# speechbrain/speechbrain

Hardware: AMD Instinct MI355X
Metric: audio-sec/s decoded (node), Conformer-L beam=10 (higher is better)
Workload: dtype f32

## Files before the change

### speechbrain_amd/csrc/ctc_prefix.hip

```cpp
#include "common.h"
#include "internal.h"

namespace {

constexpr float kNeg = sbk::kCtcNeg;
constexpr int kNegE = -(1 << 20);
constexpr int kHead = 24;

struct BF {
  float mg, mb;
  int eg, eb;
};

__device__ __forceinline__ float bf_log(float m, int e) {
  if (!(m > 0.0f)) return kNeg;
  const double v = ((double)e + (double)log2f(m)) * 0.69314718055994530942;
  return v < (double)kNeg ? kNeg : (float)v;
}
__device__ __forceinline__ void bf_exp(float x, float* m, int* e) {
  if (!(x > -1e19f)) {
    *m = 0.0f;
    *e = kNegE;
    return;
  }
  const double y = (double)x * 1.44269504088896340736;
  const double ip = floor(y);
  *m = exp2f((float)(y - ip));
  *e = (int)ip;
}

constexpr int kSeg = 32;
__device__ __host__ __forceinline__ int nseg_of(int T) { return (T + kSeg - 1) / kSeg; }
__device__ __host__ __forceinline__ int beam_pitch(int beam) { return 16 * ((beam + 15) / 16); }

template <typename Row>
__device__ __forceinline__ void build_segment_tables(Row row, int T, int lane, float* __restrict__ sg,
                                                     float* __restrict__ sb, int* __restrict__ se, int bp) {
  const int nseg = nseg_of(T);
  for (int s0 = 0; s0 < nseg; s0 += 2) {
    const int seg = s0 + (lane >> 5);
    const int t = seg * kSeg + (lane & 31);
    BF v{0.0f, 0.0f, kNegE, kNegE};
    if (seg < nseg && t < T) v = row(t);
    int e = max(v.mg > 0.0f ? v.eg : kNegE, v.mb > 0.0f ? v.eb : kNegE);
#pragma unroll
    for (int m = 16; m >= 1; m >>= 1) e = max(e, sbk::shfl_xor(e, m));
    if (seg < nseg && t < T) {
      sg[(size_t)t * bp] = sbk::fast_ldexp(v.mg, v.eg - e);
      sb[t] = sbk::fast_ldexp(v.mb, v.eb - e);
    }
    if (seg < nseg && (lane & 31) == 0) se[(size_t)seg * bp] = e;
  }
}

__global__ void __launch_bounds__(256) ctc_emissions_kernel(float* __restrict__ x, float* __restrict__ xb_log,
                                                            const int32_t* __restrict__ enc_len, int T, int V, int blank, int ldp) {
  const int b = blockIdx.y, t = blockIdx.x;
  float* row = x + ((size_t)b * T + t) * ldp;
  const bool pad = t >= enc_len[b];
  if (threadIdx.x == 0) xb_log[b * T + t] = pad ? (blank == 0 ? 0.0f : kNeg) : row[blank];
  __syncthreads();
  for (int c = threadIdx.x; c < V; c += 256) row[c] = pad ? (c == 0 ? 1.0f : 0.0f) : expf(row[c]);
}

__global__ void __launch_bounds__(256) ctc_init_kernel(const float* __restrict__ xb_log, BF* __restrict__ st,
                                                       float* __restrict__ sg, float* __restrict__ sb,
                                                       int* __restrict__ se, float* __restrict__ psi_prev, int T,
                                                       int beam) {
  SBK_DYN_LDS(float, cum);
  const int b = blockIdx.x;
  const int nseg = nseg_of(T);
  if (threadIdx.x == 0) {
    float c = 0.0f;
    for (int t = 0; t < T; ++t) {
      c += xb_log[b * T + t];
      cum[t] = c;
    }
  }
  __syncthreads();
  for (int t = threadIdx.x; t < T; t += 256) {
    BF v;
    bf_exp(cum[t], &v.mg, &v.eg);
    v.mb = v.mg;
    v.eb = v.eg;
    for (int j = 0; j < beam; ++j) st[((size_t)b * beam + j) * T + t] = v;
  }
  if (threadIdx.x < beam) psi_prev[b * beam + threadIdx.x] = 0.0f;
  __syncthreads();
  const int lane = threadIdx.x & 63, wave = threadIdx.x >> 6;
  for (int j = wave; j < beam; j += 4) {
    const size_t n = (size_t)b * beam + j;
    const BF* rowp = st + n * T;
    const int bp = beam_pitch(beam);
    build_segment_tables([&](int t) { return rowp[t]; }, T, lane, sg + (size_t)b * T * bp + j, sb + n * T,
                         se + (size_t)b * nseg * bp + j, bp);
  }
}

struct CtcStepArgs {
  const int32_t* last_tok;
  const int32_t* enc_len;
  int B, T, V, beam, prefix_len, blank, eos;
  float weight;
  int eos_floor;
  int use_eos_threshold;
  float eos_threshold, minus_inf;
  const int32_t* step_ptr;
  int min_steps;
  const int32_t* utt_min;
  int utt_beam, step;
  const int32_t* win;
  int window;
  int ldp;
};
__device__ __forceinline__ void ctc_frame_range(int prefix_len, int T, const int32_t* win, int window, int* start, int* end) {
  *start = prefix_len > 1 ? prefix_len : 1;
  *end = T;
  if (win) {
    *start = max(*start, win[0] - window);
    *end = min(T, win[1] + window);
  }
}
__device__ __forceinline__ int ctc_clip_to_length(int end, int blank, int len) { return blank == 0 ? min(end, max(len, 1)) : end; }

template <int NB, int TPT, bool NT>
__global__ void __launch_bounds__(256) ctc_score_step_kernel(CtcStepArgs a, const float* __restrict__ P,
                                                             const BF* __restrict__ st, const float* __restrict__ sg,
                                                             const int* __restrict__ se,
                                                             float* __restrict__ psi_out) {
  constexpr int BP = 16;
  constexpr int NV = (NB + 3) / 4;
  SBK_DYN_LDS(float, lds);
  if (a.step_ptr) a.prefix_len = a.step_ptr[0];
  const int b = blockIdx.y;
  const int j0 = blockIdx.z * BP, bp = beam_pitch(a.beam);
  const int T = a.T, V = a.V;
  int c[TPT], cc[TPT];
  bool c_ok[TPT];
#pragma unroll
  for (int k = 0; k < TPT; ++k) {
    c[k] = TPT == 4 ? (blockIdx.x * 256 + threadIdx.x) * 4 + k : (blockIdx.x * TPT + k) * 256 + threadIdx.x;
    c_ok[k] = c[k] < V;
    cc[k] = c_ok[k] ? c[k] : V - 1;
  }
  const int c4 = c_ok[0] ? c[0] : V - 4;
  const int nseg = nseg_of(T);
  int start, end;
  ctc_frame_range(a.prefix_len, T, a.win, a.window, &start, &end);
  end = ctc_clip_to_length(end, a.blank, a.enc_len[b]);
  const int ldp = a.ldp;
  const float* Pb = P + (size_t)b * T * ldp;
  const int last_frame = a.enc_len[b] - 1;
  float* tab = lds;
  int* segs = reinterpret_cast<int*>(lds + (size_t)T * BP);
  const int u_begin = start - 1, u_end = end - 1;
  if (a.win) {
    for (int i = threadIdx.x; i < nseg * BP; i += 256) {
      const int seg = i / BP, j = i % BP;
      int e = kNegE;
      if (j0 + j < a.beam) {
        const BF* row = st + (size_t)(b * a.beam + j0 + j) * T;
        for (int u = max(seg * kSeg, u_begin); u < min((seg + 1) * kSeg, u_end); ++u)
          if (row[u].mg > 0.0f) e = max(e, row[u].eg);
      }
      segs[i] = e;
    }
    __syncthreads();
    for (int i = threadIdx.x; i < T * BP; i += 256) {
      const int u = i / BP, j = i % BP;
      float v = 0.0f;
      if (j0 + j < a.beam && u >= u_begin && u < u_end) {
        const BF s = st[(size_t)(b * a.beam + j0 + j) * T + u];
        v = sbk::fast_ldexp(s.mg, (s.mg > 0.0f ? s.eg : kNegE) - segs[(u / kSeg) * BP + j]);
      }
      tab[i] = v;
    }
  } else {
    float4* dst = reinterpret_cast<float4*>(tab);
    for (int i = threadIdx.x; i < T * (BP / 4); i += 256)
      dst[i] = *reinterpret_cast<const float4*>(sg + ((size_t)b * T + i / (BP / 4)) * bp + j0 + 4 * (i % (BP / 4)));
    const int* es = se + (size_t)b * nseg * bp + j0;
    for (int i = threadIdx.x; i < nseg * BP; i += 256) segs[i] = es[(size_t)(i / BP) * bp + i % BP];
  }
  __syncthreads();

  float mps[TPT][NB];
  int Eps[TPT][NB];
  float part[TPT][NB];
#pragma unroll
  for (int k = 0; k < TPT; ++k) {
    const float p0 = Pb[cc[k]];
#pragma unroll
    for (int j = 0; j < NB; ++j) {
      const bool first = a.prefix_len == 0 && start == 1 && p0 > 0.0f;
      mps[k][j] = first ? p0 : 0.0f;
      Eps[k][j] = first ? 0 : kNegE;
      part[k][j] = 0.0f;
    }
  }
  constexpr int CH = 16 / TPT < 8 ? 8 : 16 / TPT;
  static_assert(kSeg % CH == 0, "ctc_score_step: chunks must tile a scale segment");
  auto fetch = [&](float (&buf)[TPT][CH], int cb) {
#pragma unroll
    for (int q = 0; q < CH; ++q) {
      const int u = cb + q;
      const bool ok = u >= u_begin && u < u_end;
      if constexpr (TPT == 4) {
        float4 v4 = make_float4(0.f, 0.f, 0.f, 0.f);
        if (ok) v4 = sbk::ld16<NT>(Pb + (size_t)(u + 1) * ldp + c4);
        buf[0][q] = v4.x; buf[1][q] = v4.y; buf[2][q] = v4.z; buf[3][q] = v4.w;
      } else {
#pragma unroll
        for (int k = 0; k < TPT; ++k) buf[k][q] = ok ? sbk::ld4<NT>(Pb + (size_t)(u + 1) * ldp + cc[k]) : 0.0f;
      }
    }
  };
  float nxt[TPT][CH];
  int cb = (u_begin / CH) * CH;
  if (cb < u_end) fetch(nxt, cb);
  for (; cb < u_end; cb += CH) {
    float cur[TPT][CH];
#pragma unroll
    for (int k = 0; k < TPT; ++k)
#pragma unroll
      for (int q = 0; q < CH; ++q) cur[k][q] = nxt[k][q];
    if (cb + CH < u_end) fetch(nxt, cb + CH);
#pragma unroll
    for (int q = 0; q < CH; ++q) {
      const float4* row = reinterpret_cast<const float4*>(tab + (size_t)min(cb + q, u_end - 1) * BP);
      float g[NV * 4];
#pragma unroll
      for (int v = 0; v < NV; ++v) {
        const float4 t4 = row[v];
        g[4 * v] = t4.x; g[4 * v + 1] = t4.y; g[4 * v + 2] = t4.z; g[4 * v + 3] = t4.w;
      }
#pragma unroll
      for (int k = 0; k < TPT; ++k)
#pragma unroll
        for (int j = 0; j < NB; ++j) part[k][j] = fmaf(g[j], cur[k][q], part[k][j]);
    }
    if (((cb + CH) % kSeg) == 0 || cb + CH >= u_end) {
      const int* es = segs + (cb / kSeg) * BP;
#pragma unroll
      for (int k = 0; k < TPT; ++k)
#pragma unroll
        for (int j = 0; j < NB; ++j) {
          const int kx = sbk::frexp_exp(part[k][j]);
          const int ep = part[k][j] > 0.0f ? es[j] + kx : kNegE;
          const float mp = sbk::fast_ldexp(part[k][j], -kx);
          const int P2 = max(Eps[k][j], ep);
          mps[k][j] = sbk::fast_ldexp(mps[k][j], Eps[k][j] - P2) + sbk::fast_ldexp(mp, ep - P2);
          Eps[k][j] = P2;
          part[k][j] = 0.0f;
        }
    }
  }
#pragma unroll
  for (int k = 0; k < TPT; ++k) {
    if (!c_ok[k]) continue;
#pragma unroll
    for (int j = 0; j < NB; ++j) {
      if (j0 + j < a.beam) {
        const int n = b * a.beam + j0 + j;
        float psi = bf_log(mps[k][j], Eps[k][j]);
        if (c[k] == a.eos) {
          const BF s = st[(size_t)n * T + last_frame];
          psi = bf_log(s.mg, s.eg);
        }
        if (c[k] == a.blank && a.eos != a.blank) psi = kNeg;
        psi_out[(size_t)n * V + c[k]] = psi;
      }
    }
  }
}

__global__ void __launch_bounds__(64) ctc_same_token_kernel(CtcStepArgs a, const float* __restrict__ P,
                                                            const BF* __restrict__ st, const float* __restrict__ sb,
                                                            const int* __restrict__ se, float* __restrict__ psi_out) {
  const int n = blockIdx.x, lane = threadIdx.x;
  if (a.step_ptr) a.prefix_len = a.step_ptr[0];
  const int b = n / a.beam, c = a.last_tok[n];
  const int T = a.T, V = a.V, nseg = nseg_of(T);
  if (c == a.eos || c == a.blank || c < 0 || c >= V) return;
  int start, end;
  ctc_frame_range(a.prefix_len, T, a.win, a.window, &start, &end);
  end = ctc_clip_to_length(end, a.blank, a.enc_len[b]);
  const float* Pb = P + (size_t)b * T * a.ldp;
  float m = 0.0f;
  int E = kNegE;
  if (lane == 0 && a.prefix_len == 0 && start == 1 && Pb[c] > 0.0f) {
    m = Pb[c];
    E = 0;
  }
  for (int u = start - 1 + lane; u < end - 1; u += 64) {
    const float bt = a.win ? st[(size_t)n * T + u].mb : sb[(size_t)n * T + u];
    const float term = bt * Pb[(size_t)(u + 1) * a.ldp + c];
    const int k = sbk::frexp_exp(term);
    const int eb = a.win ? st[(size_t)n * T + u].eb : se[((size_t)b * nseg + u / kSeg) * beam_pitch(a.beam) + n % a.beam];
    const int et = term > 0.0f ? eb + k : kNegE;
    const float mt = sbk::fast_ldexp(term, -k);
    const int E2 = max(E, et);
    m = sbk::fast_ldexp(m, E - E2) + sbk::fast_ldexp(mt, et - E2);
    E = E2;
  }
  int Emax = E;
#pragma unroll
  for (int k = 32; k >= 1; k >>= 1) Emax = max(Emax, sbk::shfl_xor(Emax, k));
  float v = sbk::fast_ldexp(m, E - Emax);
  v = sbk::wave_sum(v);
  if (lane == 0) psi_out[(size_t)n * V + c] = bf_log(v, Emax);
}

__global__ void __launch_bounds__(256) ctc_combine_kernel(CtcStepArgs a, const float* __restrict__ am,
                                                          const float* __restrict__ am_max,
                                                          const float* __restrict__ psi,
                                                          const float* __restrict__ psi_prev, float* __restrict__ comb,
                                                          const float* __restrict__ extra) {
  const int n = blockIdx.y;
  const int c = blockIdx.x * 256 + threadIdx.x;
  if (c >= a.V) return;
  float v = am[(size_t)n * a.V + c];
  if (c == a.eos) {
    const int step = a.step_ptr ? a.step_ptr[0] : a.step;
    const bool floor = a.utt_min ? step < a.utt_min[n / a.utt_beam] : (a.step_ptr ? step < a.min_steps : a.eos_floor);
    if (floor) v = a.minus_inf;
    if (a.use_eos_threshold && !(v > a.eos_threshold * am_max[n])) v = a.minus_inf;
  }
  if (extra) v = sbk::add_rn(v, extra[(size_t)n * a.V + c]);
  if (c == a.blank) v = kNeg;
  comb[(size_t)n * a.V + c] = sbk::score_ctc(v, psi[(size_t)n * a.V + c], psi_prev[n], a.weight);
}

struct AMap {
  float a, c, d, v0, v1;
  int ea, ec, ed, e0, e1;
};
struct AState {
  float nb, bl;
  int e;
};
__device__ __forceinline__ int clamp_e(int e) { return max(e, kNegE); }
__device__ __forceinline__ void norm1(float& x, int& e) {
  const int k = sbk::frexp_exp(x);
  x = sbk::fast_ldexp(x, -k);
  e = x > 0.0f ? clamp_e(e + k) : kNegE;
}
__device__ __forceinline__ void norm2(float& x, float& y, int& e) {
  const float m = fmaxf(x, y);
  const int k = sbk::frexp_exp(m);
  x = sbk::fast_ldexp(x, -k);
  y = sbk::fast_ldexp(y, -k);
  e = m > 0.0f ? e + k : kNegE;
}
__device__ __forceinline__ void bf_add(float& x, int& ex, float y, int ey) {
  const int ax = x > 0.0f ? ex : kNegE, ay = y > 0.0f ? ey : kNegE;
  const int E = max(ax, ay);
  x = sbk::fast_ldexp(x, ax - E) + sbk::fast_ldexp(y, ay - E);
  ex = E;
}
__device__ __forceinline__ AState apply_map(const AMap& m, const AState& s) {
  float x = m.a * s.nb, y = m.c * s.nb;
  int ex = clamp_e(m.ea + s.e), ey = clamp_e(m.ec + s.e);
  bf_add(x, ex, m.v0, m.e0);
  bf_add(y, ey, m.d * s.bl, clamp_e(m.ed + s.e));
  bf_add(y, ey, m.v1, m.e1);
  const int ax = x > 0.0f ? ex : kNegE, ay = y > 0.0f ? ey : kNegE;
  const int E = max(ax, ay);
  AState r{sbk::fast_ldexp(x, ax - E), sbk::fast_ldexp(y, ay - E), E};
  norm2(r.nb, r.bl, r.e);
  return r;
}
__device__ __forceinline__ AMap compose(const AMap& m2, const AMap& m1) {
  AMap r;
  r.a = m2.a * m1.a;
  r.ea = clamp_e(m2.ea + m1.ea);
  norm1(r.a, r.ea);
  r.d = m2.d * m1.d;
  r.ed = clamp_e(m2.ed + m1.ed);
  norm1(r.d, r.ed);
  r.c = m2.c * m1.a;
  r.ec = clamp_e(m2.ec + m1.ea);
  bf_add(r.c, r.ec, m2.d * m1.c, clamp_e(m2.ed + m1.ec));
  norm1(r.c, r.ec);
  r.v0 = m2.a * m1.v0;
  r.e0 = clamp_e(m2.ea + m1.e0);
  bf_add(r.v0, r.e0, m2.v0, m2.e0);
  norm1(r.v0, r.e0);
  r.v1 = m2.c * m1.v0;
  r.e1 = clamp_e(m2.ec + m1.e0);
  bf_add(r.v1, r.e1, m2.d * m1.v1, clamp_e(m2.ed + m1.e1));
  bf_add(r.v1, r.e1, m2.v1, m2.e1);
  norm1(r.v1, r.e1);
  return r;
}
__device__ __forceinline__ AMap frame_map(float pc, float pb, float mphi, int ephi) {
  AMap m;
  m.a = pc;
  m.ea = 0;
  norm1(m.a, m.ea);
  m.c = pb;
  m.ec = 0;
  norm1(m.c, m.ec);
  m.d = m.c;
  m.ed = m.ec;
  m.v0 = m.a * mphi;
  m.e0 = clamp_e(m.ea + ephi);
  norm1(m.v0, m.e0);
  m.v1 = 0.0f;
  m.e1 = kNegE;
  return m;
}
__device__ __forceinline__ AMap identity_map() { return AMap{1.0f, 0.0f, 1.0f, 0.0f, 0.0f, 0, kNegE, 0, kNegE, kNegE}; }
__device__ __forceinline__ AMap shfl_up_map(const AMap& m, int delta, int lane) {
  const int src = max(lane - delta, 0);
  AMap r;
  r.a = sbk::shfl(m.a, src);
  r.c = sbk::shfl(m.c, src);
  r.d = sbk::shfl(m.d, src);
  r.v0 = sbk::shfl(m.v0, src);
  r.v1 = sbk::shfl(m.v1, src);
  r.ea = sbk::shfl(m.ea, src);
  r.ec = sbk::shfl(m.ec, src);
  r.ed = sbk::shfl(m.ed, src);
  r.e0 = sbk::shfl(m.e0, src);
  r.e1 = sbk::shfl(m.e1, src);
  return r;
}

struct CtcAdvArgs {
  const float* P;
  const BF* st_old;
  const float* psi;
  const int32_t* parent;
  const int32_t* token;
  const int32_t* parent_last_tok;
  BF* st_new;
  float* sg_new;
  float* sb_new;
  int* se_new;
  float* psi_prev_new;
  int n_bh, T, V, beam, prefix_len, blank;
  const int32_t* step_ptr;
  const int32_t* win;
  int window;
  int ldp;
};

__global__ void __launch_bounds__(64) ctc_advance_kernel(CtcAdvArgs a) {
  SBK_DYN_LDS(float, lds);
  if (a.step_ptr) a.prefix_len = a.step_ptr[0];
  const int T = a.T;
  float* pc = lds;
  float* pb = pc + T;
  float* mph = pb + T;
  int* eph = reinterpret_cast<int*>(mph + T);
  float* onb = reinterpret_cast<float*>(eph + T);
  float* obl = onb + T;
  int* oe = reinterpret_cast<int*>(obl + T);
  const int n = blockIdx.x, lane = threadIdx.x;
  const int b = n / a.beam, p = a.parent[n], c = a.token[n];
  const bool same = a.parent_last_tok[p] == c;
  const float* Pb = a.P + (size_t)b * T * a.ldp;
  for (int tb = 0; tb < T; tb += 256) {
    float vpc[4], vpb[4];
    BF vs[4];
#pragma unroll
    for (int u = 0; u < 4; ++u) {
      const int t = min(tb + u * 64 + lane, T - 1);
      vpc[u] = Pb[(size_t)t * a.ldp + c];
      vpb[u] = Pb[(size_t)t * a.ldp + a.blank];
      vs[u] = a.st_old[(size_t)p * T + t];
    }
#pragma unroll
    for (int u = 0; u < 4; ++u) {
      const int t = tb + u * 64 + lane;
      if (t < T) {
        pc[t] = vpc[u];
        pb[t] = vpb[u];
        mph[t] = same ? vs[u].mb : vs[u].mg;
        eph[t] = same ? vs[u].eb : vs[u].eg;
      }
    }
  }
  __syncthreads();
  {
    int start, end;
    ctc_frame_range(a.prefix_len, T, a.win, a.window, &start, &end);
    const bool first = a.prefix_len == 0 && pc[0] > 0.0f;
    AState r0{first ? pc[0] : 0.0f, 0.0f, first ? 0 : kNegE};
    norm2(r0.nb, r0.bl, r0.e);
    const AState zero{0.0f, 0.0f, kNegE};
    const AState s0 = start == 1 ? r0 : zero;
    for (int t = lane; t < T; t += 64)
      if (t < start || t >= end) {
        onb[t] = t == 0 ? r0.nb : 0.0f;
        obl[t] = 0.0f;
        oe[t] = t == 0 ? r0.e : kNegE;
      }
    const int nfr = max(end - start, 0);
    const int fpl = (nfr + 63) / 64;
    const int f0 = min(start + lane * fpl, end), f1 = min(f0 + fpl, end);
    AMap mine = identity_map();
    for (int t = f0; t < f1; ++t) mine = compose(frame_map(pc[t], pb[t], mph[t - 1], eph[t - 1]), mine);
#pragma unroll
    for (int dlt = 1; dlt < 64; dlt <<= 1) {
      const AMap other = shfl_up_map(mine, dlt, lane);
      if (lane >= dlt) mine = compose(mine, other);
    }
    AMap pre = shfl_up_map(mine, 1, lane);
    if (lane == 0) pre = identity_map();
    AState st = apply_map(pre, s0);
    for (int t = f0; t < f1; ++t) {
      st = apply_map(frame_map(pc[t], pb[t], mph[t - 1], eph[t - 1]), st);
      onb[t] = st.nb;
      obl[t] = st.bl;
      oe[t] = st.e;
    }
  }
  __syncthreads();
  BF* bfrow = reinterpret_cast<BF*>(pc);
  for (int t0 = 0; t0 < T; t0 += 64) {
    const int t = t0 + lane;
    BF s{0.0f, 0.0f, kNegE, kNegE};
    if (t < T) {
      const float g = onb[t] + obl[t];
      const int kg = sbk::frexp_exp(g), kb = sbk::frexp_exp(obl[t]);
      s.mg = g > 0.0f ? sbk::fast_ldexp(g, 1 - kg) : 0.0f;
      s.eg = g > 0.0f ? oe[t] + kg - 1 : kNegE;
      s.mb = obl[t] > 0.0f ? sbk::fast_ldexp(obl[t], 1 - kb) : 0.0f;
      s.eb = obl[t] > 0.0f ? oe[t] + kb - 1 : kNegE;
      a.st_new[(size_t)n * T + t] = s;
    }
    __syncthreads();
    if (t < T) bfrow[t] = s;
  }
  __syncthreads();
  const int nseg = nseg_of(T);
  const int bp = beam_pitch(a.beam);
  build_segment_tables([&](int t) { return bfrow[t]; }, T, lane, a.sg_new + (size_t)b * T * bp + n % a.beam,
                       a.sb_new + (size_t)n * T, a.se_new + (size_t)b * nseg * bp + n % a.beam, bp);
  if (lane == 0) a.psi_prev_new[n] = a.psi[(size_t)p * a.V + c];
}

__global__ void __launch_bounds__(256) am_only_kernel(const float* __restrict__ am, float* __restrict__ comb, int V,
                                                      int eos, int eos_floor, int use_thr, float thr, float minus_inf,
                                                      const float* __restrict__ am_max,
                                                      const float* __restrict__ extra,
                                                      const int32_t* __restrict__ step_ptr, int min_steps,
                                                      const int32_t* __restrict__ utt_min, int beam, int step) {
  const int n = blockIdx.y;
  const int c = blockIdx.x * 256 + threadIdx.x;
  if (c >= V) return;
  float v = am[(size_t)n * V + c];
  if (c == eos) {
    if (step_ptr) step = step_ptr[0];
    if (utt_min ? step < utt_min[n / beam] : (step_ptr ? step < min_steps : eos_floor)) v = minus_inf;
    if (use_thr && !(v > thr * am_max[n])) v = minus_inf;
  }
  if (extra) v = sbk::add_rn(v, extra[(size_t)n * V + c]);
  comb[(size_t)n * V + c] = v;
}

__device__ __forceinline__ unsigned order_key(float x) {
  const unsigned u = __float_as_uint(x);
  return (u & 0x80000000u) ? ~u : (u | 0x80000000u);
}

__global__ void __launch_bounds__(256) row_kth_largest_kernel(const float* __restrict__ x, float* __restrict__ thr, int V,
                                                              int k) {
  __shared__ int cnt[4];
  __shared__ unsigned prefix_s;
  const float* xr = x + (size_t)blockIdx.x * V;
  unsigned prefix = 0;
  for (int bit = 31; bit >= 0; --bit) {
    const unsigned t = prefix | (1u << bit);
    int c = 0;
    for (int i = threadIdx.x; i < V; i += 256) c += order_key(xr[i]) >= t ? 1 : 0;
    c = (int)sbk::wave_sum((float)c);
    if ((threadIdx.x & 63) == 0) cnt[threadIdx.x >> 6] = c;
    __syncthreads();
    if (threadIdx.x == 0) prefix_s = ((cnt[0] + cnt[1]) + (cnt[2] + cnt[3])) >= k ? t : prefix;
    __syncthreads();
    prefix = prefix_s;
    __syncthreads();
  }
  if (threadIdx.x == 0) {
    const unsigned u = (prefix & 0x80000000u) ? (prefix & 0x7fffffffu) : ~prefix;
    thr[blockIdx.x] = __uint_as_float(u);
  }
}

__global__ void __launch_bounds__(256) ctc_partial_combine_kernel(float* __restrict__ comb, const float* __restrict__ thr,
                                                                  const float* __restrict__ psi,
                                                                  const float* __restrict__ psi_prev, int V, int blank,
                                                                  int eos, float weight, float minus_inf) {
  const int n = blockIdx.y;
  const int c = blockIdx.x * 256 + threadIdx.x;
  if (c >= V) return;
  const float base = comb[(size_t)n * V + c];
  float p = (base >= thr[n] || c == eos) ? psi[(size_t)n * V + c] : minus_inf;
  if (c == blank && eos != blank) p = minus_inf;
  comb[(size_t)n * V + c] = base + (p - psi_prev[n]) * weight;
}

__global__ void __launch_bounds__(256) row_max_kernel(const float* __restrict__ x, float* __restrict__ out, int V) {
  __shared__ float red[4];
  const float* xr = x + (size_t)blockIdx.x * V;
  float m = -INFINITY;
  for (int c = threadIdx.x; c < V; c += 256) m = fmaxf(m, xr[c]);
  m = sbk::wave_max(m);
  if ((threadIdx.x & 63) == 0) red[threadIdx.x >> 6] = m;
  __syncthreads();
  if (threadIdx.x == 0) out[blockIdx.x] = fmaxf(fmaxf(red[0], red[1]), fmaxf(red[2], red[3]));
}

}

namespace sbk {

namespace {
struct StateView {
  BF* st;
  float* sg;
  float* sb;
  int* se;
};
StateView view(float* base, int B, int beam, int T) {
  const size_t n_bh = (size_t)B * beam, bp = beam_pitch(beam);
  StateView v;
  v.st = reinterpret_cast<BF*>(base);
  v.sg = base + 4 * n_bh * T;
  v.sb = v.sg + (size_t)B * T * bp;
  v.se = reinterpret_cast<int*>(v.sb + n_bh * T);
  return v;
}
}

int ctc_psi_step(const float* P, const float* state, const int32_t* last_tok, const int32_t* enc_len, float* psi, int B,
                 int T, int V, int beam, int prefix_len, int blank, int eos, hipStream_t st, const int32_t* win, int window, int ldp);

size_t ctc_state_floats(int B, int beam, int T) {
  const size_t n_bh = (size_t)B * beam, bp = beam_pitch(beam);
  return 4 * n_bh * T + (size_t)B * T * bp + n_bh * T + (size_t)B * nseg_of(T) * bp + 16;
}

int ctc_prepare(float* x, float* xb_log, const int32_t* enc_len, float* state, float* psi_prev, int B, int T, int V,
                int beam, int blank, hipStream_t st, int ldp) {
  if (ldp < V) ldp = V;
  SBK_LAUNCH(ctc_emissions_kernel, dim3(T, B), dim3(256), 0, st, x, xb_log, enc_len, T, V, blank, ldp);
  int rc = launch_status("ctc_emissions");
  if (rc) return rc;
  StateView v = view(state, B, beam, T);
  if (hipMemsetAsync(v.sg, 0, (size_t)B * T * beam_pitch(beam) * sizeof(float), st) != hipSuccess) return fail(1, "ctc: memset");
  SBK_LAUNCH(ctc_init_kernel, dim3(B), dim3(256), (size_t)T * sizeof(float), st, (const float*)xb_log, v.st, v.sg, v.sb,
             v.se, psi_prev, T, beam);
  return launch_status("ctc_init");
}

int ctc_psi_step(const float* P, const float* state, const int32_t* last_tok, const int32_t* enc_len, float* psi, int B,
                 int T, int V, int beam, int prefix_len, int blank, int eos, hipStream_t st, const int32_t* win, int window, int ldp) {
  CtcStepArgs a{last_tok, enc_len, B, T, V, beam, prefix_len, blank, eos, 0.0f, 0, 0, 0.0f, 0.0f, g_step_ptr, 0};
  a.win = win;
  a.window = window;
  a.ldp = ldp < V ? V : ldp;
  const StateView v = view(const_cast<float*>(state), B, beam, T);
  ProfScope prof("ctc_score_step", 2.0 * B * beam * (double)T * V, 4.0 * B * (double)T * V + 4.0 * B * beam * V, st);
  constexpr int tpt = 1;
  dim3 grid(cdiv(V, 256 * tpt), B, beam_pitch(beam) / 16), block(256);
  const size_t lds = ((size_t)T * 16 + (size_t)((T + kSeg - 1) / kSeg) * 16) * sizeof(float);
  if (lds > 160 * 1024) return fail(SBK_EINVAL, "ctc_psi_step: T=%d frames need %zu B of LDS (max 160 KiB)", T, lds);
#define SBK_CTC_LAUNCH_NT(NB, TP, NT)                                                                                   \
  do {                                                                                                                  \
    if (lds > 64 * 1024 && SBK_ALLOW_DYN_LDS((ctc_score_step_kernel<NB, TP, NT>), lds) != hipSuccess)                    \
      return fail(SBK_EINVAL, "ctc_psi_step: cannot raise the LDS window to %zu B", lds);                               \
    SBK_LAUNCH((ctc_score_step_kernel<NB, TP, NT>), grid, block, lds, st, a, P, (const BF*)v.st, (const float*)v.sg,    \
               (const int*)v.se, psi);                                                                                  \
  } while (0)
#define SBK_CTC_LAUNCH_ONE(NB, TP)                                                                                      \
  do {                                                                                                                  \
    if (g_nt_mask & 4)                                                                                                  \
      SBK_CTC_LAUNCH_NT(NB, TP, true);                                                                                  \
    else                                                                                                                \
      SBK_CTC_LAUNCH_NT(NB, TP, false);                                                                                 \
  } while (0)
#define SBK_CTC_LAUNCH(NB) SBK_CTC_LAUNCH_ONE(NB, 1)
  if (beam == 1) {
    SBK_CTC_LAUNCH(1);
  } else if (beam <= 4) {
    SBK_CTC_LAUNCH(4);
  } else if (beam <= 10) {
    SBK_CTC_LAUNCH(10);
  } else {
    SBK_CTC_LAUNCH(16);
  }
#undef SBK_CTC_LAUNCH
#undef SBK_CTC_LAUNCH_ONE
#undef SBK_CTC_LAUNCH_NT
  int rc = launch_status("ctc_score_step");
  if (rc) return rc;
  SBK_LAUNCH(ctc_same_token_kernel, dim3(B * beam), dim3(64), 0, st, a, P, (const BF*)v.st, (const float*)v.sb,
             (const int*)v.se, psi);
  return launch_status("ctc_same_token");
}

int ctc_combine(const float* am, const float* am_max, const float* psi, const float* psi_prev, float* comb, int n_bh,
                int V, int blank, int eos, float weight, int eos_floor, int use_thr, float thr, float minus_inf,
                const float* extra, hipStream_t st, const int32_t* utt_min, int beam, int step) {
  CtcStepArgs a{nullptr, nullptr, 0, 0, V, 0, 0, blank, eos, weight, eos_floor, use_thr, thr, minus_inf, g_step_ptr,
                g_step_min_steps, utt_min, beam > 0 ? beam : 1, step};
  SBK_LAUNCH(ctc_combine_kernel, dim3(cdiv(V, 256), n_bh), dim3(256), 0, st, a, am, am_max, psi, psi_prev, comb, extra);
  return launch_status("ctc_combine");
}

int ctc_advance(const float* P, const float* state_old, const float* psi, const int32_t* parent, const int32_t* token,
                const int32_t* parent_last_tok, float* state_new, float* psi_prev_new, int n_bh, int T, int V, int beam,
                int prefix_len, int blank, hipStream_t st, const int32_t* win, int window, int ldp) {
  const StateView vo = view(const_cast<float*>(state_old), n_bh / beam, beam, T);
  const StateView vn = view(state_new, n_bh / beam, beam, T);
  CtcAdvArgs a{P, vo.st, psi, parent, token, parent_last_tok, vn.st, vn.sg, vn.sb, vn.se, psi_prev_new, n_bh, T, V, beam,
               prefix_len, blank, g_step_ptr, win, window, ldp < V ? V : ldp};
  const size_t lds = (size_t)7 * T * sizeof(float);
  if (lds > 64 * 1024) return fail(SBK_EINVAL, "ctc_advance: T=%d too long for the LDS window", T);
  ProfScope prof("ctc_advance", 14.0 * n_bh * T, 64.0 * n_bh * T, st);
  SBK_LAUNCH(ctc_advance_kernel, dim3(n_bh), dim3(64), lds, st, a);
  return launch_status("ctc_advance");
}

int am_only(const float* am, float* comb, int n_bh, int V, int eos, int eos_floor, int use_thr, float thr,
            float minus_inf, const float* am_max, const float* extra, hipStream_t st, const int32_t* utt_min, int beam,
            int step) {
  const int32_t* sp = g_step_ptr;
  const int min_steps = g_step_min_steps;
  SBK_LAUNCH(am_only_kernel, dim3(cdiv(V, 256), n_bh), dim3(256), 0, st, am, comb, V, eos, eos_floor, use_thr, thr,
             minus_inf, am_max, extra, sp, min_steps, utt_min, beam > 0 ? beam : 1, step);
  return launch_status("am_only");
}

int ctc_partial_combine(float* comb, float* thr, const float* psi, const float* psi_prev, int n_bh, int V, int k, int blank,
                        int eos, float weight, float minus_inf, hipStream_t st) {
  const int kk = k < 1 ? 1 : (k > V ? V : k);
  SBK_LAUNCH(row_kth_largest_kernel, dim3(n_bh), dim3(256), 0, st, (const float*)comb, thr, V, kk);
  SBK_LAUNCH(ctc_partial_combine_kernel, dim3(cdiv(V, 256), n_bh), dim3(256), 0, st, comb, (const float*)thr, psi, psi_prev,
             V, blank, eos, weight, minus_inf);
  return launch_status("ctc_partial_combine");
}

int row_max(const float* x, float* out, int rows, int V, hipStream_t st) {
  SBK_LAUNCH(row_max_kernel, dim3(rows), dim3(256), 0, st, x, out, V);
  return launch_status("row_max");
}

}


namespace {
__global__ void __launch_bounds__(256) ctc_score_delta_kernel(const float* __restrict__ psi, const float* __restrict__ psi_prev,
                                                              float* __restrict__ out, int V) {
  const int n = blockIdx.y, c = blockIdx.x * 256 + threadIdx.x;
  if (c < V) out[(size_t)n * V + c] = sbk::sub_rn(psi[(size_t)n * V + c], psi_prev[n]);
}
struct ScorerWs {
  float* phi[2];
  float* psi;
  float* psi_prev[2];
  float* xb;
};
size_t scorer_ws_floats(int B, int T, int V, int beam) {
  auto up = [](size_t n) { return (n + 63) & ~(size_t)63; };
  return 2 * up(sbk::ctc_state_floats(B, beam, T)) + up((size_t)B * beam * V) + 2 * up((size_t)B * beam) + up((size_t)B * T);
}
ScorerWs carve_scorer(void* ws, int B, int T, int V, int beam) {
  auto up = [](size_t n) { return (n + 63) & ~(size_t)63; };
  float* p = static_cast<float*>(ws);
  ScorerWs w;
  w.phi[0] = p, p += up(sbk::ctc_state_floats(B, beam, T));
  w.phi[1] = p, p += up(sbk::ctc_state_floats(B, beam, T));
  w.psi = p, p += up((size_t)B * beam * V);
  w.psi_prev[0] = p, p += up((size_t)B * beam);
  w.psi_prev[1] = p, p += up((size_t)B * beam);
  w.xb = p;
  return w;
}
}

extern "C" size_t sbk_ctc_scorer_workspace_bytes(int B, int T, int V, int beam) {
  if (B <= 0 || T <= 0 || V <= 0 || beam <= 0) return 0;
  return scorer_ws_floats(B, T, V, beam) * sizeof(float);
}

extern "C" int sbk_ctc_scorer_reset_f32(float* x, const int32_t* enc_len, void* ws, size_t ws_bytes, int B, int T, int V, int beam,
                                        int blank, sbk_stream_t stream) {
  if (B == 0) return 0;
  SBK_REQUIRE(x && enc_len && ws && B > 0 && T > 0 && V > 0 && beam > 0 && blank >= 0 && blank < V, "ctc_scorer_reset: bad arguments");
  SBK_REQUIRE(ws_bytes >= sbk_ctc_scorer_workspace_bytes(B, T, V, beam) && sbk::aligned16(ws) && sbk::aligned16(x),
              "ctc_scorer_reset: workspace too small (%zu B) or unaligned", ws_bytes);
  hipStream_t st = sbk::as_stream(stream);
  const ScorerWs w = carve_scorer(ws, B, T, V, beam);
  if (hipMemsetAsync(w.phi[1], 0, sbk::ctc_state_floats(B, beam, T) * sizeof(float), st) != hipSuccess)
    return sbk::fail(1, "ctc_scorer_reset: memset");
  return sbk::ctc_prepare(x, w.xb, enc_len, w.phi[0], w.psi_prev[0], B, T, V, beam, blank, st, V);
}

extern "C" int sbk_ctc_scorer_score_f32(const float* x, const int32_t* enc_len, void* ws, size_t ws_bytes, const int32_t* inp_tokens,
                                        int step, const int32_t* attn_window, int ctc_window_size, float* scores, int B, int T, int V,
                                        int beam, int blank, int eos, sbk_stream_t stream) {
  if (B == 0) return 0;
  SBK_REQUIRE(x && enc_len && ws && inp_tokens && scores && B > 0 && T > 0 && V > 0 && beam > 0 && step >= 0, "ctc_scorer_score: bad arguments");
  SBK_REQUIRE(ws_bytes >= sbk_ctc_scorer_workspace_bytes(B, T, V, beam), "ctc_scorer_score: workspace too small");
  SBK_REQUIRE(ctc_window_size >= 0 && (ctc_window_size == 0 || attn_window), "ctc_scorer_score: a window needs the {min, max} attention peaks");
  hipStream_t st = sbk::as_stream(stream);
  const ScorerWs w = carve_scorer(ws, B, T, V, beam);
  const int cur = step & 1;
  const int32_t* win = ctc_window_size > 0 ? attn_window : nullptr;
  int rc = sbk::ctc_psi_step(x, w.phi[cur], inp_tokens, enc_len, w.psi, B, T, V, beam, step, blank, eos, st, win, ctc_window_size, V);
  if (rc) return rc;
  SBK_LAUNCH(ctc_score_delta_kernel, dim3(sbk::cdiv(V, 256), B * beam), dim3(256), 0, st, (const float*)w.psi,
             (const float*)w.psi_prev[cur], scores, V);
  return sbk::launch_status("ctc_score_delta");
}

extern "C" int sbk_ctc_scorer_permute_f32(const float* x, void* ws, size_t ws_bytes, const int32_t* parent, const int32_t* token,
                                          const int32_t* parent_last_tok, int step, const int32_t* attn_window, int ctc_window_size,
                                          int B, int T, int V, int beam, int blank, sbk_stream_t stream) {
  if (B == 0) return 0;
  SBK_REQUIRE(x && ws && parent && token && parent_last_tok && B > 0 && T > 0 && V > 0 && beam > 0 && step >= 0, "ctc_scorer_permute: bad arguments");
  SBK_REQUIRE(ws_bytes >= sbk_ctc_scorer_workspace_bytes(B, T, V, beam), "ctc_scorer_permute: workspace too small");
  SBK_REQUIRE(ctc_window_size >= 0 && (ctc_window_size == 0 || attn_window), "ctc_scorer_permute: a window needs the {min, max} attention peaks");
  const ScorerWs w = carve_scorer(ws, B, T, V, beam);
  const int cur = step & 1;
  return sbk::ctc_advance(x, w.phi[cur], w.psi, parent, token, parent_last_tok, w.phi[cur ^ 1], w.psi_prev[cur ^ 1], B * beam, T, V,
                          beam, step, blank, sbk::as_stream(stream), ctc_window_size > 0 ? attn_window : nullptr, ctc_window_size, V);
}

extern "C" int sbk_prof_ctc_psi_repeat_f32(float* P_logsoftmax, const int32_t* enc_len, const int32_t* last_tok,
                                           float* psi, float* work, int B, int T, int V, int beam, int prefix_len,
                                           int iters, float* us_per_launch, sbk_stream_t stream) {
  SBK_REQUIRE(P_logsoftmax && enc_len && last_tok && psi && work && us_per_launch && iters > 0, "psi_repeat: bad arguments");
  hipStream_t st = sbk::as_stream(stream);
  float* state = work;
  float* xb = work + sbk::ctc_state_floats(B, beam, T);
  float* psi_prev = xb + (size_t)B * T;
  int rc = sbk::ctc_prepare(P_logsoftmax, xb, enc_len, state, psi_prev, B, T, V, beam, 0, st, V);
  hipEvent_t e0, e1;
  if (hipEventCreate(&e0) != hipSuccess || hipEventCreate(&e1) != hipSuccess) return sbk::fail(1, "event create");
  for (int i = 0; i < 2 && !rc; ++i)
    rc = sbk::ctc_psi_step(P_logsoftmax, state, last_tok, enc_len, psi, B, T, V, beam, prefix_len, 0, 2, st, nullptr, 0, V);
  (void)hipEventRecord(e0, st);
  for (int i = 0; i < iters && !rc; ++i)
    rc = sbk::ctc_psi_step(P_logsoftmax, state, last_tok, enc_len, psi, B, T, V, beam, prefix_len, 0, 2, st, nullptr, 0, V);
  (void)hipEventRecord(e1, st);
  (void)hipEventSynchronize(e1);
  float ms = 0.0f;
  (void)hipEventElapsedTime(&ms, e0, e1);
  *us_per_launch = ms * 1000.0f / iters;
  return rc;
}
```

### speechbrain_amd/csrc/search.hip

```cpp
#include <limits.h>

#include "common.h"
#include "internal.h"

namespace {
struct AsyncPoll {
  static constexpr int kRing = 4;
  int32_t* host = nullptr;
  hipEvent_t ev[kRing] = {};
  int issued = 0;
  bool ok = false;
  bool begin() {
    if (!ok) {
      if (hipHostMalloc(reinterpret_cast<void**>(&host), kRing * sizeof(int32_t), 0) != hipSuccess) return false;
      for (int i = 0; i < kRing; ++i)
        if (hipEventCreateWithFlags(&ev[i], hipEventDisableTiming) != hipSuccess) return false;
      ok = true;
    }
    for (int j = issued > kRing ? issued - kRing : 0; j < issued; ++j) (void)hipEventSynchronize(ev[j % kRing]);
    issued = 0;
    return true;
  }
  int poll(const int32_t* counter_dev, int target, hipStream_t st) {
    const int k = issued % kRing;
    if (hipMemcpyAsync(host + k, counter_dev, sizeof(int32_t), hipMemcpyDeviceToHost, st) != hipSuccess ||
        hipEventRecord(ev[k], st) != hipSuccess)
      return -1;
    ++issued;
    if (issued >= 3) {
      const int j = (issued - 3) % kRing;
      if (hipEventSynchronize(ev[j]) != hipSuccess) return -1;
      if (host[j] >= target) return 1;
    }
    for (int q = issued >= 2 ? issued - 2 : 0; q < issued; ++q)
      if (hipEventQuery(ev[q % kRing]) == hipSuccess && host[q % kRing] >= target) return 1;
    return 0;
  }
};
thread_local AsyncPoll g_poll;
}

namespace sbk {
int embed_pos(const int32_t* tok, const float* emb, const float* pe_row, float* x, int n, int d, float scale,
              hipStream_t st);
int self_attn_step(const float* qkv, float* kcache, float* vcache, const int32_t* kv_slot, float* out, int n, int d,
                   int H, int step, int nslot, int Lmax, hipStream_t st, const int32_t* key_tok = nullptr,
                   int key_stride = 0, int key_shift = 0, int key_first = 0, int pad_idx = 0, int group = 1);
int cross_attn_step(const float* q, const float* kv, const int32_t* enc_len, float* out, float* part, int B, int T,
                    int d, int H, int beam, hipStream_t st);
size_t cross_attn_partial_floats(int B, int T, int H, int Dh, int beam);
int log_softmax_rows(const float* x, float* out, int rows, int V, float temperature, float weight, hipStream_t st,
                     const float* bias = nullptr, const float* bias2 = nullptr, int ld = 0);
int ctc_prepare(float* x, float* xb_log, const int32_t* enc_len, float* state, float* psi_prev, int B, int T, int V,
                int beam, int blank, hipStream_t st, int ldp = 0);
size_t ctc_state_floats(int B, int beam, int T);
int ctc_psi_step(const float* P, const float* state, const int32_t* last_tok, const int32_t* enc_len, float* psi, int B,
                 int T, int V, int beam, int prefix_len, int blank, int eos, hipStream_t st, const int32_t* win = nullptr,
                 int window = 0, int ldp = 0);
int cross_attn_avg_probs(const float* q, const float* kv, const int32_t* enc_len, float* out, int n, int T, int d, int H,
                         int beam, hipStream_t st);
int ctc_combine(const float* am, const float* am_max, const float* psi, const float* psi_prev, float* comb, int n_bh,
                int V, int blank, int eos, float weight, int eos_floor, int use_thr, float thr, float minus_inf,
                const float* extra, hipStream_t st, const int32_t* utt_min = nullptr, int beam = 1, int step = 0);
int ctc_advance(const float* x, const float* phi_old, const float* psi, const int32_t* parent, const int32_t* token,
                const int32_t* parent_last_tok, float* phi_new, float* psi_prev_new, int n_bh, int T, int V, int beam,
                int prefix_len, int blank, hipStream_t st, const int32_t* win = nullptr, int window = 0, int ldp = 0);
int am_only(const float* am, float* comb, int n_bh, int V, int eos, int eos_floor, int use_thr, float thr,
            float minus_inf, const float* am_max, const float* extra, hipStream_t st, const int32_t* utt_min = nullptr,
            int beam = 1, int step = 0);
int row_max(const float* x, float* out, int rows, int V, hipStream_t st);
int ctc_partial_combine(float* comb, float* thr, const float* psi, const float* psi_prev, int n_bh, int V, int k, int blank,
                        int eos, float weight, float minus_inf, hipStream_t st);
int g_score_fused = 1;
}

namespace {

struct SideStream {
  hipStream_t s = nullptr;
  hipEvent_t fork = nullptr, join = nullptr;
};
SideStream* side_stream() {
  static thread_local SideStream ss;
  if (!ss.s) {
    if (hipStreamCreateWithFlags(&ss.s, hipStreamNonBlocking) != hipSuccess) return nullptr;
    if (hipEventCreateWithFlags(&ss.fork, hipEventDisableTiming) != hipSuccess ||
        hipEventCreateWithFlags(&ss.join, hipEventDisableTiming) != hipSuccess)
      return nullptr;
  }
  return &ss;
}

constexpr int kMaxBeam = 16;
constexpr int kMaxBeamLarge = 128;

struct Cand {
  float v;
  int i;
};
__device__ __forceinline__ bool better(float v, int i, float v2, int i2) { return v > v2 || (v == v2 && i < i2); }

template <typename Load>
__device__ __forceinline__ void block_topk(int total, int k, float* out_val, int32_t* out_idx, Load load) {
  __shared__ float lv[kMaxBeam][256];
  __shared__ int li[kMaxBeam][256];
  __shared__ float wv[4][kMaxBeam];
  __shared__ int wi[4][kMaxBeam];
  const int tid = threadIdx.x, lane = tid & 63, wave = tid >> 6;
  float vals[kMaxBeam];
  int ids[kMaxBeam];
#pragma unroll
  for (int s = 0; s < kMaxBeam; ++s) {
    vals[s] = -INFINITY;
    ids[s] = INT_MAX;
  }
  for (int e = tid; e < total; e += 256) {
    float vn;
    int id;
    load(e, vn, id);
    if (vn != vn) continue;
    if (better(vn, id, vals[kMaxBeam - 1], ids[kMaxBeam - 1])) {
      float cv = vn;
      int ci = id;
#pragma unroll
      for (int s = 0; s < kMaxBeam; ++s) {
        if (better(cv, ci, vals[s], ids[s])) {
          const float tv = vals[s];
          const int ti = ids[s];
          vals[s] = cv;
          ids[s] = ci;
          cv = tv;
          ci = ti;
        }
      }
    }
  }
#pragma unroll
  for (int s = 0; s < kMaxBeam; ++s) {
    lv[s][tid] = vals[s];
    li[s][tid] = ids[s];
  }
  int hp = 0;
  for (int r = 0; r < k; ++r) {
    float v = hp < kMaxBeam ? lv[hp][tid] : -INFINITY;
    int i = hp < kMaxBeam ? li[hp][tid] : INT_MAX;
    const int mine = i;
    sbk::wave_argmax(v, i);
    if (lane == 0) {
      wv[wave][r] = v;
      wi[wave][r] = i;
    }
    if (hp < kMaxBeam && mine == i && i != INT_MAX) ++hp;
  }
  __syncthreads();
  if (wave == 0) {
    float v = -INFINITY;
    int i = INT_MAX;
    if (lane < 4 * k) {
      v = wv[lane / k][lane % k];
      i = wi[lane / k][lane % k];
    }
    for (int r = 0; r < k; ++r) {
      float bv = v;
      int bi = i;
      sbk::wave_argmax(bv, bi);
      if (lane == 0) {
        out_val[r] = bv;
        out_idx[r] = bi;
      }
      if (i == bi && bi != INT_MAX) {
        v = -INFINITY;
        i = INT_MAX;
      }
    }
  }
}

constexpr int kTopkChunks = 16;

__global__ void __launch_bounds__(256) beam_topk_stage1_kernel(const float* __restrict__ comb,
                                                               const float* __restrict__ seq, float* __restrict__ pval,
                                                               int32_t* __restrict__ pidx, int V, int beam, float norm,
                                                               const int32_t* __restrict__ step_ptr, int step,
                                                               const int32_t* __restrict__ utt_max) {
  if (step_ptr && norm > 0.0f) norm = (float)(step_ptr[0] + 1);
  if (step_ptr) step = step_ptr[0];
  const int b = blockIdx.y, ch = blockIdx.x;
  if (utt_max && step >= utt_max[b]) return;
  const int total = beam * V;
  const int len = (total + kTopkChunks - 1) / kTopkChunks;
  const int e0 = ch * len, n = max(0, min(len, total - e0));
  const float* cb = comb + (size_t)b * total;
  const float* sq = seq + b * beam;
  block_topk(n, beam, pval + ((size_t)b * kTopkChunks + ch) * kMaxBeam, pidx + ((size_t)b * kTopkChunks + ch) * kMaxBeam,
             [&](int e, float& v, int& id) {
               id = e0 + e;
               v = sbk::score_cand(sq[id / V], cb[id], norm);
             });
}

__global__ void __launch_bounds__(256) beam_topk_stage2_kernel(const float* __restrict__ pval,
                                                               const int32_t* __restrict__ pidx,
                                                               float* __restrict__ out_val,
                                                               int32_t* __restrict__ out_idx, int beam,
                                                               const int32_t* __restrict__ step_ptr, int step,
                                                               const int32_t* __restrict__ utt_max, int nchunks) {
  const int b = blockIdx.x;
  if (step_ptr) step = step_ptr[0];
  if (utt_max && step >= utt_max[b]) return;
  const float* pv = pval + (size_t)b * kTopkChunks * kMaxBeam;
  const int32_t* pi = pidx + (size_t)b * kTopkChunks * kMaxBeam;
  block_topk(nchunks * kMaxBeam, beam, out_val + b * beam, out_idx + b * beam, [&](int e, float& v, int& id) {
    const bool ok = (e % kMaxBeam) < beam;
    v = ok ? pv[e] : -INFINITY;
    id = ok ? pi[e] : INT_MAX;
  });
  __syncthreads();
  if (threadIdx.x < beam && out_idx[b * beam + threadIdx.x] == INT_MAX) out_idx[b * beam + threadIdx.x] = 0;
}

struct ScoreArgs {
  const float* logits;
  const float* bias;
  const float* bias2;
  float* am;
  const float* psi;
  const float* psi_prev;
  const float* extra;
  const float* seq;
  float* pval;
  int32_t* pidx;
  const int32_t* step_ptr;
  const int32_t* utt_min;
  const int32_t* utt_max;
  int V, beam, step, min_steps, eos_floor, use_thr, eos, blank;
  float inv_temp, w, ctc_weight, thr, minus_inf, norm;
};

template <int NPT>
__global__ void __launch_bounds__(256) score_topk_row_kernel(ScoreArgs a) {
  __shared__ float red[4];
  __shared__ float wv[4][kMaxBeam];
  __shared__ int wi[4][kMaxBeam];
  const int n = blockIdx.x, tid = threadIdx.x, lane = tid & 63, wave = tid >> 6;
  const int V = a.V, b = n / a.beam, j = n % a.beam;
  const int step = a.step_ptr ? a.step_ptr[0] : a.step;
  if (a.utt_max && step >= a.utt_max[b]) return;
  float norm = a.norm;
  if (a.step_ptr && norm > 0.0f) norm = (float)(step + 1);
  const size_t ro = (size_t)n * V;
  float x[NPT], ps[NPT], ex[NPT];
#pragma unroll
  for (int i = 0; i < NPT; ++i) x[i] = a.logits[ro + min(tid + 256 * i, V - 1)];
  if (a.psi) {
#pragma unroll
    for (int i = 0; i < NPT; ++i) ps[i] = a.psi[ro + min(tid + 256 * i, V - 1)];
  }
  if (a.extra) {
#pragma unroll
    for (int i = 0; i < NPT; ++i) ex[i] = a.extra[ro + min(tid + 256 * i, V - 1)];
  }
  float m = -INFINITY;
#pragma unroll
  for (int i = 0; i < NPT; ++i) {
    const int c = tid + 256 * i, cl = min(c, V - 1);
    const float v = sbk::ls_logit(x[i], a.bias ? a.bias[cl] : 0.0f, a.bias2 ? a.bias2[cl] : 0.0f, a.inv_temp);
    x[i] = c < V ? v : -INFINITY;
    if (c < V) m = fmaxf(m, v);
  }
  m = sbk::wave_max(m);
  if (lane == 0) red[wave] = m;
  __syncthreads();
  m = fmaxf(fmaxf(red[0], red[1]), fmaxf(red[2], red[3]));
  __syncthreads();
  float s = 0.0f;
#pragma unroll
  for (int i = 0; i < NPT; ++i)
    if (tid + 256 * i < V) s = sbk::add_rn(s, expf(sbk::sub_rn(x[i], m)));
  s = sbk::wave_sum(s);
  if (lane == 0) red[wave] = s;
  __syncthreads();
  const float lse = sbk::add_rn(m, logf((red[0] + red[1]) + (red[2] + red[3])));
  __syncthreads();
  float am_max = -INFINITY;
#pragma unroll
  for (int i = 0; i < NPT; ++i) {
    const int c = tid + 256 * i;
    if (c < V) {
      x[i] = sbk::ls_out(x[i], lse, a.w);
      a.am[ro + c] = x[i];
      am_max = fmaxf(am_max, x[i]);
    }
  }
  if (a.use_thr) {
    am_max = sbk::wave_max(am_max);
    if (lane == 0) red[wave] = am_max;
    __syncthreads();
    am_max = fmaxf(fmaxf(red[0], red[1]), fmaxf(red[2], red[3]));
  }
  const float sq = a.seq[n];
  const float pp = a.psi ? a.psi_prev[n] : 0.0f;
  unsigned dead = 0;
  float bv = -INFINITY;
  int bi = INT_MAX;
#pragma unroll
  for (int i = 0; i < NPT; ++i) {
    const int c = tid + 256 * i;
    if (c >= V) {
      dead |= 1u << i;
      continue;
    }
    float v = x[i];
    if (c == a.eos) {
      const bool floor = a.utt_min ? step < a.utt_min[b] : (a.step_ptr ? step < a.min_steps : a.eos_floor != 0);
      if (floor) v = a.minus_inf;
      if (a.use_thr && !(v > a.thr * am_max)) v = a.minus_inf;
    }
    if (a.extra) v = sbk::add_rn(v, ex[i]);
    if (a.psi) {
      if (c == a.blank) v = sbk::kCtcNeg;
      v = sbk::score_ctc(v, ps[i], pp, a.ctc_weight);
    }
    v = sbk::score_cand(sq, v, norm);
    x[i] = v;
    if (v != v) {
      dead |= 1u << i;
      continue;
    }
    const int id = j * V + c;
    if (better(v, id, bv, bi)) {
      bv = v;
      bi = id;
    }
  }
  const int k = a.beam;
  for (int r = 0; r < k; ++r) {
    float v = bv;
    int i2 = bi;
    sbk::wave_argmax(v, i2);
    if (lane == 0) {
      wv[wave][r] = v;
      wi[wave][r] = i2;
    }
    if (bi == i2 && i2 != INT_MAX) {
      dead |= 1u << ((bi - j * V - tid) >> 8);
      bv = -INFINITY;
      bi = INT_MAX;
#pragma unroll
      for (int i = 0; i < NPT; ++i) {
        const int id = j * V + tid + 256 * i;
        if (!((dead >> i) & 1u) && better(x[i], id, bv, bi)) {
          bv = x[i];
          bi = id;
        }
      }
    }
  }
  __syncthreads();
  if (wave == 0) {
    float v = -INFINITY;
    int i2 = INT_MAX;
    if (lane < 4 * k) {
      v = wv[lane / k][lane % k];
      i2 = wi[lane / k][lane % k];
    }
    float* ov_ = a.pval + ((size_t)b * kTopkChunks + j) * kMaxBeam;
    int32_t* oi_ = a.pidx + ((size_t)b * kTopkChunks + j) * kMaxBeam;
    for (int r = 0; r < k; ++r) {
      float wbv = v;
      int wbi = i2;
      sbk::wave_argmax(wbv, wbi);
      if (lane == 0) {
        ov_[r] = wbv;
        oi_[r] = wbi;
      }
      if (i2 == wbi && wbi != INT_MAX) {
        v = -INFINITY;
        i2 = INT_MAX;
      }
    }
  }
}

__device__ __forceinline__ unsigned order_key(float v) {
  const unsigned u = __float_as_uint(v);
  return (u & 0x80000000u) ? ~u : (u | 0x80000000u);
}

__global__ void __launch_bounds__(1024) beam_topk_large_kernel(const float* __restrict__ comb,
                                                               const float* __restrict__ seq,
                                                               float* __restrict__ out_val,
                                                               int32_t* __restrict__ out_idx, int V, int beam,
                                                               float norm, const int32_t* __restrict__ step_ptr,
                                                               int step, const int32_t* __restrict__ utt_max) {
  if (step_ptr && norm > 0.0f) norm = (float)(step_ptr[0] + 1);
  if (step_ptr) step = step_ptr[0];
  if (utt_max && step >= utt_max[blockIdx.x]) return;
  __shared__ int hist[256];
  __shared__ unsigned s_prefix;
  __shared__ int s_remaining, s_count, s_eq_base;
  __shared__ int scan[1024];
  __shared__ float wv[kMaxBeamLarge];
  __shared__ int wi[kMaxBeamLarge];
  const int b = blockIdx.x, tid = threadIdx.x;
  const int total = beam * V;
  const float* cb = comb + (size_t)b * total;
  const float* sq = seq + b * beam;
  auto value = [&](int e) {
    const float x = sq[e / V] + cb[e];
    const float v = norm > 0.0f ? x / norm : x;
    return v != v ? -INFINITY : v;
  };
  if (tid == 0) {
    s_prefix = 0u;
    s_remaining = beam;
  }
  for (int pass = 0; pass < 4; ++pass) {
    const int shift = 24 - 8 * pass;
    if (tid < 256) hist[tid] = 0;
    __syncthreads();
    const unsigned prefix = s_prefix;
    for (int e = tid; e < total; e += 1024) {
      const unsigned k = order_key(value(e));
      if (pass == 0 || (k >> (shift + 8)) == prefix) atomicAdd(&hist[(k >> shift) & 255u], 1);
    }
    __syncthreads();
    if (tid == 0) {
      int rem = s_remaining, d = 255;
      for (; d > 0; --d) {
        if (hist[d] >= rem) break;
        rem -= hist[d];
      }
      s_remaining = rem;
      s_prefix = (prefix << 8) | (unsigned)d;
    }
    __syncthreads();
  }
  const unsigned thr = s_prefix;
  const int need_eq = s_remaining;
  if (tid == 0) {
    s_count = 0;
    s_eq_base = 0;
  }
  for (int i = tid; i < kMaxBeamLarge; i += 1024) {
    wv[i] = -INFINITY;
    wi[i] = INT_MAX;
  }
  __syncthreads();
  __shared__ int s_ties;
  if (tid == 0) s_ties = 0;
  __syncthreads();
  for (int e = tid; e < total; e += 1024) {
    const float v = value(e);
    const unsigned k = order_key(v);
    if (k > thr) {
      const int slot = atomicAdd(&s_count, 1);
      if (slot < kMaxBeamLarge) {
        wv[slot] = v;
        wi[slot] = e;
      }
    } else if (k == thr) {
      const int t = atomicAdd(&s_ties, 1);
      if (t < 1024) scan[t] = e;
    }
  }
  __syncthreads();
  const int n_ties = s_ties;
  if (n_ties <= 1024) {
    if (tid < n_ties) {
      const int e = scan[tid];
      int rank = 0;
      for (int q = 0; q < n_ties; ++q) rank += scan[q] < e;
      if (rank < need_eq) {
        const int slot = atomicAdd(&s_count, 1);
        if (slot < kMaxBeamLarge) {
          wv[slot] = value(e);
          wi[slot] = e;
        }
      }
    }
    __syncthreads();
  } else {
    __syncthreads();
    for (int e0 = 0; e0 < total; e0 += 1024) {
      const int e = e0 + tid;
      const int is_eq = (e < total && order_key(value(e)) == thr) ? 1 : 0;
      scan[tid] = is_eq;
      __syncthreads();
      for (int off = 1; off < 1024; off <<= 1) {
        const int add = tid >= off ? scan[tid - off] : 0;
        __syncthreads();
        scan[tid] += add;
        __syncthreads();
      }
      const int eq_rank = s_eq_base + scan[tid] - is_eq;
      if (is_eq && eq_rank < need_eq) {
        const int slot = atomicAdd(&s_count, 1);
        if (slot < kMaxBeamLarge) {
          wv[slot] = value(e);
          wi[slot] = e;
        }
      }
      __syncthreads();
      if (tid == 0) s_eq_base += scan[1023];
      __syncthreads();
      if (s_eq_base >= need_eq) break;
    }
    __syncthreads();
  }
  for (int size = 2; size <= kMaxBeamLarge; size <<= 1) {
    for (int stride = size >> 1; stride > 0; stride >>= 1) {
      if (tid < kMaxBeamLarge) {
        const int partner = tid ^ stride;
        if (partner > tid) {
          const bool desc = (tid & size) == 0;
          const bool first_better = better(wv[tid], wi[tid], wv[partner], wi[partner]);
          if (desc != first_better) {
            const float tv = wv[tid];
            const int ti = wi[tid];
            wv[tid] = wv[partner];
            wi[tid] = wi[partner];
            wv[partner] = tv;
            wi[partner] = ti;
          }
        }
      }
      __syncthreads();
    }
  }
  if (tid < beam) {
    out_val[b * beam + tid] = wv[tid];
    out_idx[b * beam + tid] = wi[tid] == INT_MAX ? 0 : wi[tid];
  }
}

struct BeamState {
  int32_t* seq[2];
  float* lp[2];
  int32_t* kv_slot[2];
  int32_t* tokens[2];
  float* seq_scores;
  float* cand_val;
  int32_t* cand_idx;
  int32_t* parent;
  int32_t* fin_count;
  int32_t* fin_seq;
  float* fin_lp;
  int32_t* fin_len;
  float* fin_score;
  int32_t* n_full;
  int pos_off;
};

__global__ void step_inc_kernel(int32_t* step) { step[0] += 1; }

__global__ void beam_init_kernel(BeamState s, int B, int beam, int bos) {
  const int n = blockIdx.x * blockDim.x + threadIdx.x;
  if (n == 0) {
    s.n_full[0] = 0;
    s.n_full[1] = 0;
  }
  if (n < B) s.fin_count[n] = 0;
  if (n >= B * beam) return;
  s.tokens[0][n] = bos;
  s.seq_scores[n] = (n % beam == 0) ? 0.0f : -INFINITY;
}

__global__ void kv_prompt_init_kernel(BeamState s, int n, int Lmax, int pos_off) {
  const int i = blockIdx.x * blockDim.x + threadIdx.x;
  if (i >= n * pos_off) return;
  const int h = i / pos_off, p = i % pos_off;
  s.kv_slot[0][(size_t)h * Lmax + p] = h;
  s.kv_slot[1][(size_t)h * Lmax + p] = h;
}
__global__ void prompt_col_kernel(const int32_t* __restrict__ prompt, int32_t* __restrict__ col, int n, int beam, int P, int p) {
  const int h = blockIdx.x * blockDim.x + threadIdx.x;
  if (h < n) col[h] = prompt[(size_t)(h / beam) * P + p];
}
__global__ void probe_pick_kernel(const float* __restrict__ probe, float* __restrict__ out, int B, int beam) {
  const int b = blockIdx.x * blockDim.x + threadIdx.x;
  if (b < B) out[b] = probe[(size_t)b * beam];
}

__device__ __forceinline__ void beam_update_body(const BeamState& s, const float* __restrict__ am, int cur, int step, int V,
                                                 int beam, int Lmax, int eos, int length_norm,
                                                 const int32_t* __restrict__ utt_max) {
  __shared__ int h_src[kMaxBeamLarge];
  __shared__ int h_dst[kMaxBeamLarge];
  __shared__ int h_n;
  const int b = blockIdx.x, tid = threadIdx.x;
  const int nxt = cur ^ 1;
  if (utt_max && step >= utt_max[b]) {
    for (int idx = tid; idx < beam * (step + 1); idx += 256) {
      const int j = idx / (step + 1), p = idx % (step + 1);
      const size_t o = ((size_t)b * beam + j) * Lmax + p;
      s.seq[nxt][o] = p < step ? s.seq[cur][o] : 0;
      s.lp[nxt][o] = p < step ? s.lp[cur][o] : 0.0f;
      s.kv_slot[nxt][o + s.pos_off] = p < step ? s.kv_slot[cur][o + s.pos_off] : b * beam + j;
    }
    if (tid < beam) {
      s.tokens[nxt][b * beam + tid] = s.tokens[cur][b * beam + tid];
      s.parent[b * beam + tid] = b * beam + tid;
    }
    return;
  }
  for (int idx = tid; idx < beam * (step + 1); idx += 256) {
    const int j = idx / (step + 1), p = idx % (step + 1);
    const int n = b * beam + j;
    const int cand = s.cand_idx[n];
    const int pred = b * beam + cand / V, tok = cand % V;
    const size_t o = (size_t)n * Lmax + p, po = (size_t)pred * Lmax + p;
    if (p < step) {
      s.seq[nxt][o] = s.seq[cur][po];
      s.lp[nxt][o] = s.lp[cur][po];
      s.kv_slot[nxt][o + s.pos_off] = s.kv_slot[cur][po + s.pos_off];
    } else {
      s.seq[nxt][o] = tok;
      s.lp[nxt][o] = am[(size_t)pred * V + tok];
      s.kv_slot[nxt][o + s.pos_off] = pred;
      s.tokens[nxt][n] = tok;
      s.parent[n] = pred;
    }
  }
  if (tid == 0) {
    int cnt = s.fin_count[b], nh = 0;
    const int before = cnt;
    for (int j = 0; j < beam; ++j) {
      const int n = b * beam + j;
      const int tok = s.cand_idx[n] % V;
      const float score = s.cand_val[n];
      if (tok == eos && cnt < beam) {
        h_src[nh] = j;
        h_dst[nh] = cnt;
        ++nh;
        s.fin_len[b * beam + cnt] = step + 1;
        s.fin_score[b * beam + cnt] = score;
        ++cnt;
      }
      s.seq_scores[n] = tok == eos ? -INFINITY : (length_norm ? score * (float)(step + 1) : score);
    }
    s.fin_count[b] = cnt;
    h_n = nh;
    if (cnt == beam && before < beam) atomicAdd(s.n_full, 1);
  }
  __syncthreads();
  for (int k = 0; k < h_n; ++k) {
    const int n = b * beam + h_src[k];
    const int cand = s.cand_idx[n];
    const int pred = b * beam + cand / V, tok = cand % V;
    const size_t fo = ((size_t)b * beam + h_dst[k]) * Lmax;
    for (int p = tid; p <= step; p += 256) {
      s.fin_seq[fo + p] = p < step ? s.seq[cur][(size_t)pred * Lmax + p] : tok;
      s.fin_lp[fo + p] = p < step ? s.lp[cur][(size_t)pred * Lmax + p] : am[(size_t)pred * V + tok];
    }
  }
}

__global__ void __launch_bounds__(256) beam_update_kernel(BeamState s, const float* __restrict__ am, int cur, int step,
                                                          int V, int beam, int Lmax, int eos, int length_norm,
                                                          const int32_t* __restrict__ step_ptr,
                                                          const int32_t* __restrict__ utt_max) {
  if (step_ptr) step = step_ptr[0];
  beam_update_body(s, am, cur, step, V, beam, Lmax, eos, length_norm, utt_max);
}

__global__ void __launch_bounds__(256) beam_merge_update_kernel(BeamState s, const float* __restrict__ pval,
                                                                const int32_t* __restrict__ pidx,
                                                                const float* __restrict__ am, int cur, int step, int V,
                                                                int beam, int Lmax, int eos, int length_norm,
                                                                const int32_t* __restrict__ step_ptr,
                                                                const int32_t* __restrict__ utt_max, int nchunks) {
  const int b = blockIdx.x;
  if (step_ptr) step = step_ptr[0];
  if (!(utt_max && step >= utt_max[b])) {
    const float* pv = pval + (size_t)b * kTopkChunks * kMaxBeam;
    const int32_t* pi = pidx + (size_t)b * kTopkChunks * kMaxBeam;
    block_topk(nchunks * kMaxBeam, beam, s.cand_val + b * beam, s.cand_idx + b * beam, [&](int e, float& v, int& id) {
      const bool ok = (e % kMaxBeam) < beam;
      v = ok ? pv[e] : -INFINITY;
      id = ok ? pi[e] : INT_MAX;
    });
    __syncthreads();
    if (threadIdx.x < beam && s.cand_idx[b * beam + threadIdx.x] == INT_MAX) s.cand_idx[b * beam + threadIdx.x] = 0;
    __syncthreads();
  }
  beam_update_body(s, am, cur, step, V, beam, Lmax, eos, length_norm, utt_max);
}

__global__ void __launch_bounds__(256) beam_finalize_kernel(BeamState s, int cur, int steps_done, int beam, int Lmax,
                                                            int Lout, int topk, int32_t* __restrict__ out_tok,
                                                            int32_t* __restrict__ out_len, float* __restrict__ out_score,
                                                            float* __restrict__ out_lp,
                                                            const int32_t* __restrict__ utt_max,
                                                            int32_t* __restrict__ out_longest) {
  if (utt_max) steps_done = min(steps_done, utt_max[blockIdx.x]);
  __shared__ float e_score[kMaxBeamLarge];
  __shared__ int e_src[kMaxBeamLarge];
  __shared__ int sel[kMaxBeamLarge];
  __shared__ int n_entries;
  const int b = blockIdx.x, tid = threadIdx.x;
  if (tid == 0) {
    int cnt = s.fin_count[b];
    for (int f = 0; f < cnt; ++f) {
      e_score[f] = s.fin_score[b * beam + f];
      e_src[f] = f;
    }
    int longest = 0;
    for (int f = 0; f < cnt; ++f) longest = max(longest, s.fin_len[b * beam + f]);
    if (steps_done > 0) {
      if (cnt < beam) longest = max(longest, steps_done);
      for (int j = 0; j < beam && cnt < beam; ++j, ++cnt) {
        e_score[cnt] = s.cand_val[b * beam + j];
        e_src[cnt] = -(j + 1);
      }
    }
    atomicMax(&s.n_full[1], longest);
    if (out_longest) out_longest[b] = longest;
    n_entries = cnt;
    for (int r = 0; r < topk; ++r) {
      int bi = -1;
      for (int e = 0; e < cnt; ++e) {
        bool used = false;
        for (int q = 0; q < r; ++q) used |= sel[q] == e;
        if (!used && (bi < 0 || e_score[e] > e_score[bi])) bi = e;
      }
      sel[r] = bi;
    }
  }
  __syncthreads();
  for (int r = 0; r < topk; ++r) {
    const int e = sel[r];
    const size_t row = (size_t)b * topk + r;
    int ntok = 0;
    if (e >= 0) ntok = e_src[e] < 0 ? steps_done : s.fin_len[b * beam + e_src[e]];
    const int len = ntok > 0 ? ntok - 1 : 0;
    if (tid == 0) {
      out_score[row] = e >= 0 ? e_score[e] : 0.0f;
      out_len[row] = len;
    }
    for (int p = tid; p < Lout; p += 256) {
      int tok = 0;
      float lp = 0.0f;
      if (e >= 0 && p < ntok) {
        const size_t o = e_src[e] < 0 ? ((size_t)b * beam + (-e_src[e] - 1)) * Lmax + p
                                      : ((size_t)b * beam + e_src[e]) * Lmax + p;
        tok = e_src[e] < 0 ? s.seq[cur][o] : s.fin_seq[o];
        lp = e_src[e] < 0 ? s.lp[cur][o] : s.fin_lp[o];
      }
      out_tok[row * Lout + p] = (topk > 1 ? p < ntok : p < len) ? tok : 0;
      out_lp[row * Lout + p] = lp;
    }
  }
}

__global__ void __launch_bounds__(256) greedy_pick_kernel(const float* __restrict__ logits, int32_t* __restrict__ tok_out,
                                                          int32_t* __restrict__ ended, int32_t* __restrict__ hyp,
                                                          float* __restrict__ score, int32_t* __restrict__ n_ended,
                                                          int V, int k, int Lmax, int eos,
                                                          const float* __restrict__ bias1,
                                                          const float* __restrict__ bias2) {
  __shared__ float wv[4];
  __shared__ int wi[4];
  __shared__ float red[4];
  __shared__ float row_lse;
  const int i = blockIdx.x, tid = threadIdx.x;
  const float* x = logits + (size_t)i * V;
  auto at = [&](int c) { return x[c] + (bias1 ? bias1[c] : 0.0f) + (bias2 ? bias2[c] : 0.0f); };
  float v = -INFINITY;
  int a = INT_MAX;
  for (int c = tid; c < V; c += 256) {
    const float xc = at(c);
    if (better(xc, c, v, a)) {
      v = xc;
      a = c;
    }
  }
#pragma unroll
  for (int m = 32; m >= 1; m >>= 1) {
    const float ov = sbk::shfl_xor(v, m);
    const int oi = sbk::shfl_xor(a, m);
    if (better(ov, oi, v, a)) {
      v = ov;
      a = oi;
    }
  }
  if ((tid & 63) == 0) {
    wv[tid >> 6] = v;
    wi[tid >> 6] = a;
  }
  __syncthreads();
  float bv = wv[0];
  int bi = wi[0];
  for (int w = 1; w < 4; ++w)
    if (better(wv[w], wi[w], bv, bi)) {
      bv = wv[w];
      bi = wi[w];
    }
  float se = 0.0f;
  for (int c = tid; c < V; c += 256) se += expf(at(c) - bv);
  se = sbk::wave_sum(se);
  if ((tid & 63) == 0) red[tid >> 6] = se;
  __syncthreads();
  if (tid == 0) {
    row_lse = logf((red[0] + red[1]) + (red[2] + red[3]));
    const int was = ended[i];
    const int now = was | (bi == eos);
    if (now && !was) atomicAdd(n_ended, 1);
    ended[i] = now;
    hyp[(size_t)i * Lmax + k] = now ? eos : bi;
    score[(size_t)i * Lmax + k] = now ? 0.0f : -row_lse;
    tok_out[i] = now ? eos : bi;
  }
}

__global__ void greedy_init_kernel(int32_t* tok, int32_t* ended, int32_t* n_ended, int32_t* kv_slot, int n, int Lmax,
                                   int bos) {
  const int i = blockIdx.x * blockDim.x + threadIdx.x;
  if (i == 0) *n_ended = 0;
  if (i >= n) return;
  tok[i] = bos;
  ended[i] = 0;
  for (int p = 0; p < Lmax; ++p) kv_slot[(size_t)i * Lmax + p] = i;
}

__global__ void __launch_bounds__(256) softmax_prob_kernel(const float* __restrict__ logits, float* __restrict__ out, int V,
                                                           int token) {
  __shared__ float red[4];
  const int i = blockIdx.x, tid = threadIdx.x;
  const float* x = logits + (size_t)i * V;
  float m = -INFINITY;
  for (int c = tid; c < V; c += 256) m = fmaxf(m, x[c]);
  m = sbk::wave_max(m);
  if ((tid & 63) == 0) red[tid >> 6] = m;
  __syncthreads();
  m = fmaxf(fmaxf(red[0], red[1]), fmaxf(red[2], red[3]));
  __syncthreads();
  float se = 0.0f;
  for (int c = tid; c < V; c += 256) se += expf(x[c] - m);
  se = sbk::wave_sum(se);
  if ((tid & 63) == 0) red[tid >> 6] = se;
  __syncthreads();
  if (tid == 0) out[i] = expf(x[token] - m) / ((red[0] + red[1]) + (red[2] + red[3]));
}

__global__ void copy_rows_kernel(const float* __restrict__ src, float* __restrict__ dst, int n, int d, long dst_stride) {
  const int i = blockIdx.x;
  for (int c = threadIdx.x; c < d; c += blockDim.x) dst[(size_t)i * dst_stride + c] = src[(size_t)i * d + c];
}

struct Carver {
  char* p;
  size_t used;
  bool dry;
  template <typename T>
  T* take(size_t n) {
    const size_t bytes = (n * sizeof(T) + 255) & ~(size_t)255;
    T* r = dry ? nullptr : reinterpret_cast<T*>(p + used);
    used += bytes;
    return r;
  }
};

struct DecoderBufs {
  float *x, *h, *qkv, *ctx, *q, *ff, *logits;
  float* splitk;
  size_t splitk_floats;
  float* xpart;
  int32_t* pbar;
  mutable int pseq;
  mutable int pgrid;
  float* ckv[64];
  float *kcache[64], *vcache[64];
};

void carve_decoder(Carver& c, DecoderBufs& d, const sbk_decoder_weights* W, int n, int B, int T, int Lmax) {
  const int dm = W->d_model;
  d.x = c.take<float>((size_t)n * dm);
  d.h = c.take<float>((size_t)n * dm);
  d.qkv = c.take<float>((size_t)n * 3 * dm);
  d.ctx = c.take<float>((size_t)n * dm);
  d.q = c.take<float>((size_t)n * dm);
  d.ff = c.take<float>((size_t)n * W->d_ffn);
  d.logits = c.take<float>((size_t)n * W->vocab);
  d.splitk_floats = (size_t)4 * n * (size_t)dm;
  d.splitk = c.take<float>(d.splitk_floats);
  d.xpart = c.take<float>(sbk::cross_attn_partial_floats(B, T, W->nhead, dm / W->nhead, n / (B > 0 ? B : 1)) + 64);
  d.pbar = c.take<int32_t>(64 + 512 + 256);
  d.pseq = 0;
  d.pgrid = 0;
  for (int l = 0; l < W->n_layers; ++l) {
    d.ckv[l] = c.take<float>((size_t)B * T * 2 * dm);
    d.kcache[l] = c.take<float>((size_t)Lmax * n * dm);
    d.vcache[l] = c.take<float>((size_t)Lmax * n * dm);
  }
}

#define SBK_HIP(expr)                                                              \
  do {                                                                             \
    hipError_t e__ = (expr);                                                       \
    if (e__ != hipSuccess) return sbk::fail((int)e__, "%s: %s", #expr, hipGetErrorString(e__)); \
  } while (0)

static inline int ctc_pitch(int V) { return (V + 31) & ~31; }

#define SBK_TRY(expr)        \
  do {                       \
    int rc__ = (expr);       \
    if (rc__) return rc__;   \
  } while (0)

int project_memory(const sbk_decoder_weights* W, const DecoderBufs& d, const float* enc, int B, int T,
                   hipStream_t st) {
  const int dm = W->d_model;
  SBK_HIP(hipMemsetAsync(d.pbar, 0, (64 + 512 + 256) * sizeof(int32_t), st));
  d.pseq = 0;
  d.pgrid = 0;
  for (int l = 0; l < W->n_layers; ++l) {
    const sbk_decoder_layer& L = W->layers[l];
    float* dst = d.ckv[l];
    int rc = -1;
    if (L.ca_kv_w3 && sbk::x3_routed(B * T, 2 * dm, dm))
      rc = sbk::gemm_nt_x3(enc, dm, L.ca_kv_w3, L.ca_in_b + dm, nullptr, 0, dst, 2 * dm, B * T, 2 * dm, dm, SBK_ACT_NONE, 1.0f,
                           nullptr, 0, st);
    if (rc == -1)
      rc = sbk::gemm_nt(enc, dm, L.ca_in_w + (size_t)dm * dm, dm, L.ca_in_b + dm, nullptr, 0, dst, 2 * dm, B * T, 2 * dm, dm,
                        SBK_ACT_NONE, 1.0f, nullptr, 0, st);
    SBK_TRY(rc);
  }
  return 0;
}

int decoder_step(const sbk_decoder_weights* W, const DecoderBufs& d, const int32_t* tokens, const int32_t* kv_slot,
                 const int32_t* enc_len, int step, int n, int B, int T, int beam, int Lmax, bool want_logits,
                 hipStream_t st) {
  const int dm = W->d_model, H = W->nhead;
  if (!sbk::g_step_ptr && sbk::persist_eligible(W, n, B, beam, Lmax)) {
    const int rc = sbk::decoder_step_persist(W, tokens, kv_slot, enc_len, d.x, d.qkv, d.ctx, d.q, d.ff, d.h, d.logits, d.kcache,
                                             d.vcache, d.ckv, d.pbar, d.pseq, &d.pgrid, step, n, B, T, beam, Lmax, want_logits, st);
    if (rc == 0) {
      ++d.pseq;
      return 0;
    }
    if (rc != -1) return rc;
  }
  const float emb_scale = W->emb_scale > 0.0f ? W->emb_scale : sqrtf((float)dm);
  SBK_TRY(sbk::embed_pos(tokens, W->emb, W->pe + (size_t)step * dm, d.x, n, dm, emb_scale, st));
  auto x3r = [&](const float* A, int lda, const uint16_t* WP, const float* b, const float* R, float* C, int N, int K, int act) -> int {
    if (!WP || !sbk::x3r_routed(n, N, K)) return -1;
    return sbk::gemm_nt_x3r(A, lda, WP, b, R, N, C, N, n, N, K, act, 1.0f, st);
  };
  auto biases_aligned = [](const sbk_decoder_layer& L) {
    return sbk::aligned16(L.sa_in_b) && sbk::aligned16(L.sa_out_b) && sbk::aligned16(L.ca_in_b) && sbk::aligned16(L.ca_out_b) &&
           sbk::aligned16(L.ff1_b) && sbk::aligned16(L.ff2_b) && sbk::aligned16(L.sa_in_bf) && sbk::aligned16(L.ca_q_bf) &&
           sbk::aligned16(L.ff1_bf);
  };
  for (int l = 0; l < W->n_layers; ++l) {
    const sbk_decoder_layer& L = W->layers[l];
    if (L.sa_in_wp && L.sa_out_wp && L.ca_q_wp && L.ca_out_wp && L.ff1_wp && L.ff2_wp && sbk::x3r_routed(n, dm, dm) &&
        sbk::x3r_routed(n, dm, W->d_ffn) && biases_aligned(L)) {
      const bool lnf = sbk::x3r_ln_routed(dm) && L.sa_in_wfp && L.sa_in_bf && L.ca_q_wfp && L.ca_q_bf && L.ff1_wfp && L.ff1_bf;
      auto ln_proj = [&](const float* g_, const float* b_, const uint16_t* WFP, const float* bfold, const uint16_t* WP, const float* bias,
                         float* C, int N, int act) -> int {
        if (lnf) return sbk::gemm_ln_nt_x3r(d.x, dm, WFP, bfold, nullptr, 0, C, N, n, N, dm, W->ln_eps, act, 1.0f, st);
        SBK_TRY(sbk::layernorm(d.x, g_, b_, d.h, n, dm, W->ln_eps, SBK_ACT_NONE, st));
        return x3r(d.h, dm, WP, bias, nullptr, C, N, dm, act);
      };
      SBK_TRY(ln_proj(L.ln1_g, L.ln1_b, L.sa_in_wfp, L.sa_in_bf, L.sa_in_wp, L.sa_in_b, d.qkv, 3 * dm, SBK_ACT_NONE));
      SBK_TRY(sbk::self_attn_step(d.qkv, d.kcache[l], d.vcache[l], kv_slot, d.ctx, n, dm, H, step, n, Lmax, st, nullptr, 0, 0,
                                  0, 0, beam));
      SBK_TRY(x3r(d.ctx, dm, L.sa_out_wp, L.sa_out_b, d.x, d.x, dm, dm, SBK_ACT_NONE));
      SBK_TRY(ln_proj(L.ln2_g, L.ln2_b, L.ca_q_wfp, L.ca_q_bf, L.ca_q_wp, L.ca_in_b, d.q, dm, SBK_ACT_NONE));
      SBK_TRY(sbk::cross_attn_step(d.q, d.ckv[l], enc_len, d.ctx, d.xpart, B, T, dm, H, beam, st));
      SBK_TRY(x3r(d.ctx, dm, L.ca_out_wp, L.ca_out_b, d.x, d.x, dm, dm, SBK_ACT_NONE));
      SBK_TRY(ln_proj(L.ln3_g, L.ln3_b, L.ff1_wfp, L.ff1_bf, L.ff1_wp, L.ff1_b, d.ff, W->d_ffn, W->ffn_act));
      SBK_TRY(x3r(d.ff, W->d_ffn, L.ff2_wp, L.ff2_b, d.x, d.x, dm, W->d_ffn, SBK_ACT_NONE));
      continue;
    }
    int frc = L.sa_in_wf ? sbk::gemm_ln_nt(d.x, dm, L.sa_in_wf, dm, L.sa_in_bf, nullptr, 0, d.qkv, 3 * dm, n, 3 * dm, dm,
                                           W->ln_eps, SBK_ACT_NONE, 1.0f, st)
                         : -1;
    if (frc > 0 || frc < -1) return frc;
    if (frc == -1) {
      SBK_TRY(sbk::layernorm(d.x, L.ln1_g, L.ln1_b, d.h, n, dm, W->ln_eps, SBK_ACT_NONE, st));
      SBK_TRY(sbk::gemm_nt_ws(d.h, dm, L.sa_in_w, dm, L.sa_in_b, nullptr, 0, d.qkv, 3 * dm, n, 3 * dm, dm, SBK_ACT_NONE,
                              1.0f, nullptr, 0, d.splitk, d.splitk_floats, st));
    }
    SBK_TRY(sbk::self_attn_step(d.qkv, d.kcache[l], d.vcache[l], kv_slot, d.ctx, n, dm, H, step, n, Lmax, st, nullptr, 0, 0,
                                0, 0, beam));
    SBK_TRY(sbk::gemm_nt_ws(d.ctx, dm, L.sa_out_w, dm, L.sa_out_b, d.x, dm, d.x, dm, n, dm, dm, SBK_ACT_NONE, 1.0f, nullptr,
                         0, d.splitk, d.splitk_floats, st));
    frc = L.ca_q_wf ? sbk::gemm_ln_nt(d.x, dm, L.ca_q_wf, dm, L.ca_q_bf, nullptr, 0, d.q, dm, n, dm, dm, W->ln_eps,
                                      SBK_ACT_NONE, 1.0f, st)
                    : -1;
    if (frc > 0 || frc < -1) return frc;
    if (frc == -1) {
      SBK_TRY(sbk::layernorm(d.x, L.ln2_g, L.ln2_b, d.h, n, dm, W->ln_eps, SBK_ACT_NONE, st));
      SBK_TRY(sbk::gemm_nt_ws(d.h, dm, L.ca_in_w, dm, L.ca_in_b, nullptr, 0, d.q, dm, n, dm, dm, SBK_ACT_NONE, 1.0f, nullptr,
                              0, d.splitk, d.splitk_floats, st));
    }
    SBK_TRY(sbk::cross_attn_step(d.q, d.ckv[l], enc_len, d.ctx, d.xpart, B, T, dm, H, beam, st));
    SBK_TRY(sbk::gemm_nt_ws(d.ctx, dm, L.ca_out_w, dm, L.ca_out_b, d.x, dm, d.x, dm, n, dm, dm, SBK_ACT_NONE, 1.0f, nullptr,
                         0, d.splitk, d.splitk_floats, st));
    frc = L.ff1_wf ? sbk::gemm_ln_nt(d.x, dm, L.ff1_wf, dm, L.ff1_bf, nullptr, 0, d.ff, W->d_ffn, n, W->d_ffn, dm, W->ln_eps,
                                     W->ffn_act, 1.0f, st)
                   : -1;
    if (frc > 0 || frc < -1) return frc;
    if (frc == -1) {
      SBK_TRY(sbk::layernorm(d.x, L.ln3_g, L.ln3_b, d.h, n, dm, W->ln_eps, SBK_ACT_NONE, st));
      SBK_TRY(sbk::gemm_nt_ws(d.h, dm, L.ff1_w, dm, L.ff1_b, nullptr, 0, d.ff, W->d_ffn, n, W->d_ffn, dm, W->ffn_act, 1.0f,
                              nullptr, 0, d.splitk, d.splitk_floats, st));
    }
    SBK_TRY(sbk::gemm_nt_ws(d.ff, W->d_ffn, L.ff2_w, W->d_ffn, L.ff2_b, d.x, dm, d.x, dm, n, dm, W->d_ffn, SBK_ACT_NONE, 1.0f,
                         nullptr, 0, d.splitk, d.splitk_floats, st));
  }
  if (want_logits && W->seq_wf) {
    const int frc = sbk::gemm_ln_nt(d.x, dm, W->seq_wf, dm, W->seq_bf, nullptr, 0, d.logits, W->vocab, n, W->vocab, dm,
                                    W->ln_eps, SBK_ACT_NONE, 1.0f, st);
    if (frc != -1) return frc;
  }
  if (want_logits && W->seq_wfp && W->seq_bf && sbk::x3r_ln_routed(dm) && sbk::x3r_routed(n, W->vocab, dm) &&
      (W->vocab < 4096 || sbk::g_x3r_ln == 2)) {
    const int rc = sbk::gemm_ln_nt_x3r(d.x, dm, W->seq_wfp, W->seq_bf, nullptr, 0, d.logits, W->vocab, n, W->vocab, dm, W->ln_eps,
                                       SBK_ACT_NONE, 1.0f, st);
    if (rc != -1) return rc;
  }
  SBK_TRY(sbk::layernorm(d.x, W->final_ln_g, W->final_ln_b, d.h, n, dm, W->ln_eps, SBK_ACT_NONE, st));
  if (want_logits) {
    int rc = x3r(d.h, dm, W->seq_wp, W->seq_b, nullptr, d.logits, W->vocab, dm, SBK_ACT_NONE);
    if (rc == -1 && W->seq_w3 && sbk::x3_routed(n, W->vocab, dm))
      rc = sbk::gemm_nt_x3(d.h, dm, W->seq_w3, W->seq_b, nullptr, 0, d.logits, W->vocab, n, W->vocab, dm, SBK_ACT_NONE, 1.0f,
                           nullptr, 0, st);
    if (rc == -1)
      rc = sbk::gemm_nt_ws(d.h, dm, W->seq_w, dm, W->seq_b, nullptr, 0, d.logits, W->vocab, n, W->vocab, dm, SBK_ACT_NONE, 1.0f,
                           nullptr, 0, d.splitk, d.splitk_floats, st);
    SBK_TRY(rc);
  }
  return 0;
}

struct LmBufs {
  float *x, *t, *h, *qkv, *ctx, *ff, *logits;
  float* splitk;
  size_t splitk_floats;
  float *kcache[64], *vcache[64];
};

void carve_lm(Carver& c, LmBufs& d, const sbk_lm_weights* LM, int n, int Lmax) {
  const int dm = LM->d_model;
  d.x = c.take<float>((size_t)n * dm);
  d.t = c.take<float>((size_t)n * dm);
  d.h = c.take<float>((size_t)n * dm);
  d.qkv = c.take<float>((size_t)n * 3 * dm);
  d.ctx = c.take<float>((size_t)n * dm);
  d.ff = c.take<float>((size_t)n * LM->d_ffn);
  d.logits = c.take<float>((size_t)n * LM->vocab);
  d.splitk_floats = (size_t)4 * n * (size_t)dm;
  d.splitk = c.take<float>(d.splitk_floats);
  for (int l = 0; l < LM->n_layers; ++l) {
    d.kcache[l] = c.take<float>((size_t)Lmax * n * dm);
    d.vcache[l] = c.take<float>((size_t)Lmax * n * dm);
  }
}

int check_lm(const sbk_lm_weights* LM) {
  SBK_REQUIRE(LM && LM->layers && LM->emb && LM->pe && LM->final_ln_g && LM->final_ln_b && LM->out0_w && LM->out0_b &&
                  LM->out_ln_g && LM->out_ln_b && LM->out2_w && LM->out2_b,
              "lm weights: null pointer");
  SBK_REQUIRE(LM->n_layers > 0 && LM->n_layers <= 64 && LM->d_model > 0 && LM->nhead > 0 &&
                  LM->d_model % LM->nhead == 0 && LM->vocab > 0,
              "lm weights: bad shape");
  return 0;
}

int lm_step(const sbk_lm_weights* LM, const LmBufs& d, const int32_t* tokens, const int32_t* kv_slot,
            const int32_t* key_tok, int key_stride, int key_shift, int key_first, int step, int n, int Lmax,
            hipStream_t st) {
  const int dm = LM->d_model, H = LM->nhead, ff = LM->d_ffn;
  const float eps = LM->ln_eps;
  auto gemm = [&](const float* A, int lda, const float* Wt, const float* b, const float* R, float* C, int N, int K,
                  int act) {
    return sbk::gemm_nt_ws(A, lda, Wt, K, b, R, R ? N : 0, C, N, n, N, K, act, 1.0f, nullptr, 0, d.splitk,
                           d.splitk_floats, st);
  };
  SBK_TRY(sbk::embed_pos(tokens, LM->emb, LM->pe + (size_t)step * dm, d.x, n, dm, sqrtf((float)dm), st));
  for (int l = 0; l < LM->n_layers; ++l) {
    const sbk_lm_layer& L = LM->layers[l];
    if (LM->normalize_before) {
      SBK_TRY(sbk::layernorm(d.x, L.ln1_g, L.ln1_b, d.h, n, dm, eps, SBK_ACT_NONE, st));
      SBK_TRY(gemm(d.h, dm, L.in_w, L.in_b, nullptr, d.qkv, 3 * dm, dm, SBK_ACT_NONE));
      SBK_TRY(sbk::self_attn_step(d.qkv, d.kcache[l], d.vcache[l], kv_slot, d.ctx, n, dm, H, step, n, Lmax, st, key_tok,
                                  key_stride, key_shift, key_first, LM->pad_idx));
      SBK_TRY(gemm(d.ctx, dm, L.out_w, L.out_b, d.x, d.x, dm, dm, SBK_ACT_NONE));
      SBK_TRY(sbk::layernorm(d.x, L.ln2_g, L.ln2_b, d.h, n, dm, eps, SBK_ACT_NONE, st));
      SBK_TRY(gemm(d.h, dm, L.ff1_w, L.ff1_b, nullptr, d.ff, ff, dm, LM->ffn_act));
      SBK_TRY(gemm(d.ff, ff, L.ff2_w, L.ff2_b, d.x, d.x, dm, ff, SBK_ACT_NONE));
    } else {
      SBK_TRY(gemm(d.x, dm, L.in_w, L.in_b, nullptr, d.qkv, 3 * dm, dm, SBK_ACT_NONE));
      SBK_TRY(sbk::self_attn_step(d.qkv, d.kcache[l], d.vcache[l], kv_slot, d.ctx, n, dm, H, step, n, Lmax, st, key_tok,
                                  key_stride, key_shift, key_first, LM->pad_idx));
      SBK_TRY(gemm(d.ctx, dm, L.out_w, L.out_b, d.x, d.t, dm, dm, SBK_ACT_NONE));
      SBK_TRY(sbk::layernorm(d.t, L.ln1_g, L.ln1_b, d.x, n, dm, eps, SBK_ACT_NONE, st));
      SBK_TRY(gemm(d.x, dm, L.ff1_w, L.ff1_b, nullptr, d.ff, ff, dm, LM->ffn_act));
      SBK_TRY(gemm(d.ff, ff, L.ff2_w, L.ff2_b, d.x, d.t, dm, ff, SBK_ACT_NONE));
      SBK_TRY(sbk::layernorm(d.t, L.ln2_g, L.ln2_b, d.x, n, dm, eps, SBK_ACT_NONE, st));
    }
  }
  SBK_TRY(sbk::layernorm(d.x, LM->final_ln_g, LM->final_ln_b, d.h, n, dm, eps, SBK_ACT_NONE, st));
  SBK_TRY(gemm(d.h, dm, LM->out0_w, LM->out0_b, nullptr, d.t, dm, dm, SBK_ACT_NONE));
  SBK_TRY(sbk::layernorm(d.t, LM->out_ln_g, LM->out_ln_b, d.h, n, dm, eps, SBK_ACT_NONE, st));
  SBK_TRY(gemm(d.h, dm, LM->out2_w, LM->out2_b, nullptr, d.logits, LM->vocab, dm, SBK_ACT_NONE));
  return 0;
}

int check_weights(const sbk_decoder_weights* W) {
  SBK_REQUIRE(W && W->layers && W->emb && W->pe && W->final_ln_g && W->final_ln_b, "decoder weights: null pointer");
  SBK_REQUIRE(W->n_layers > 0 && W->n_layers <= 64 && W->d_model > 0 && W->nhead > 0 && W->d_model % W->nhead == 0,
              "decoder weights: bad shape");
  return 0;
}

struct BeamBufs {
  BeamState s;
  float *am, *comb, *psi, *am_max, *ctc_x, *ctc_xb, *phi[2], *psi_prev[2];
  float* topk_val;
  int32_t* topk_idx;
  float* attn_avg;
  float* peak_val[2];
  int32_t* peak_pos[2];
  int32_t* win;
};

__global__ void __launch_bounds__(256) attn_peak_kernel(const float* __restrict__ probs, const float* __restrict__ old_val,
                                                        const int32_t* __restrict__ old_pos,
                                                        const int32_t* __restrict__ parent, float* __restrict__ new_val,
                                                        int32_t* __restrict__ new_pos, int32_t* __restrict__ win, int T,
                                                        int step) {
  __shared__ int lo_s[4], hi_s[4];
  const int n = blockIdx.x, tid = threadIdx.x;
  const int p = step > 0 ? parent[n] : n;
  int lo = INT_MAX, hi = INT_MIN;
  for (int t = tid; t < T; t += 256) {
    float v = step > 0 ? old_val[(size_t)p * T + t] : -1.0f;
    int pos = step > 0 ? old_pos[(size_t)p * T + t] : 0;
    const float a = probs[(size_t)n * T + t];
    if (a > v) {
      v = a;
      pos = step;
    }
    new_val[(size_t)n * T + t] = v;
    new_pos[(size_t)n * T + t] = pos;
    lo = min(lo, pos);
    hi = max(hi, pos);
  }
  for (int m = 32; m >= 1; m >>= 1) {
    lo = min(lo, sbk::shfl_xor(lo, m));
    hi = max(hi, sbk::shfl_xor(hi, m));
  }
  if ((tid & 63) == 0) {
    lo_s[tid >> 6] = lo;
    hi_s[tid >> 6] = hi;
  }
  __syncthreads();
  if (tid == 0) {
    atomicMin(&win[2 * step], min(min(lo_s[0], lo_s[1]), min(lo_s[2], lo_s[3])));
    atomicMax(&win[2 * step + 1], max(max(hi_s[0], hi_s[1]), max(hi_s[2], hi_s[3])));
  }
}
__global__ void win_init_kernel(int32_t* win, int steps) {
  const int i = blockIdx.x * blockDim.x + threadIdx.x;
  if (i < steps) {
    win[2 * i] = INT_MAX;
    win[2 * i + 1] = INT_MIN;
  }
}

void carve_beam(Carver& c, BeamBufs& b, int B, int beam, int T, int V, int Lmax, bool ctc, int window = 0) {
  const size_t n = (size_t)B * beam;
  for (int k = 0; k < 2; ++k) {
    b.s.seq[k] = c.take<int32_t>(n * Lmax);
    b.s.lp[k] = c.take<float>(n * Lmax);
    b.s.kv_slot[k] = c.take<int32_t>(n * Lmax);
    b.s.tokens[k] = c.take<int32_t>(n);
  }
  b.s.seq_scores = c.take<float>(n);
  b.s.cand_val = c.take<float>(n);
  b.s.cand_idx = c.take<int32_t>(n);
  b.s.parent = c.take<int32_t>(n);
  b.s.fin_count = c.take<int32_t>(B);
  b.s.fin_seq = c.take<int32_t>(n * Lmax);
  b.s.fin_lp = c.take<float>(n * Lmax);
  b.s.fin_len = c.take<int32_t>(n);
  b.s.fin_score = c.take<float>(n);
  b.s.n_full = c.take<int32_t>(64);
  b.am = c.take<float>(n * V);
  b.comb = c.take<float>(n * V);
  b.am_max = c.take<float>(n);
  b.topk_val = c.take<float>((size_t)B * kTopkChunks * kMaxBeam);
  b.topk_idx = c.take<int32_t>((size_t)B * kTopkChunks * kMaxBeam);
  if (ctc) {
    b.psi = c.take<float>(n * V);
    b.ctc_x = c.take<float>((size_t)B * T * ctc_pitch(V));
    b.ctc_xb = c.take<float>((size_t)B * T);
    for (int k = 0; k < 2; ++k) {
      b.phi[k] = c.take<float>(sbk::ctc_state_floats(B, beam, T));
      b.psi_prev[k] = c.take<float>(n);
    }
    if (window > 0) {
      b.attn_avg = c.take<float>(n * T);
      for (int k = 0; k < 2; ++k) {
        b.peak_val[k] = c.take<float>(n * T);
        b.peak_pos[k] = c.take<int32_t>(n * T);
      }
      b.win = c.take<int32_t>((size_t)2 * Lmax);
    }
  }
}

}

extern "C" size_t sbk_beam_search_workspace_bytes(const sbk_decoder_weights* W, const sbk_search_config* cfg, int B,
                                                  int T) {
  if (!W || !cfg) return 0;
  Carver c{nullptr, 0, true};
  DecoderBufs d;
  BeamBufs bb;
  const int Lmax = (cfg->max_steps > 0 ? cfg->max_steps : 1) + (cfg->prompt && cfg->prompt_len > 1 ? cfg->prompt_len - 1 : 0);
  carve_decoder(c, d, W, B * cfg->beam, B, T, Lmax);
  carve_beam(c, bb, B, cfg->beam, T, W->vocab, Lmax, cfg->ctc_weight > 0.0f, cfg->ctc_window_size);
  if (cfg->lm && cfg->lm_weight != 0.0f) {
    LmBufs lb;
    carve_lm(c, lb, cfg->lm, B * cfg->beam, Lmax);
  }
  return c.used + 256;
}

extern "C" int sbk_beam_search_f32(const sbk_decoder_weights* W, const sbk_search_config* cfg, const float* enc,
                                   const int32_t* enc_len, const float* ctc_w, const float* ctc_b, void* workspace,
                                   size_t workspace_bytes, int32_t* out_tokens, int32_t* out_len, float* out_score,
                                   float* out_logp, int32_t* out_max_len, int32_t* out_longest, int32_t* host_flag,
                                   int32_t* steps_run, int B, int T, sbk_stream_t stream) {
  SBK_TRY(check_weights(W));
  if (B == 0) {
    if (steps_run) *steps_run = 0;
    return 0;
  }
  SBK_REQUIRE(cfg && enc && enc_len && workspace && out_tokens && out_len && out_score && out_logp, "beam_search: null");
  SBK_REQUIRE(W->seq_w && W->seq_b, "beam_search: seq_lin weights missing");
  SBK_REQUIRE(cfg->beam >= 1 && cfg->beam <= kMaxBeamLarge, "beam_search: beam %d outside [1,%d]", cfg->beam,
              kMaxBeamLarge);
  const int pos_off = cfg->prompt && cfg->prompt_len > 1 ? cfg->prompt_len - 1 : 0;
  SBK_REQUIRE(pos_off + cfg->max_steps <= W->max_len, "beam_search: %d prompt + %d steps exceed the positional table (%d)",
              pos_off, cfg->max_steps, W->max_len);
  SBK_REQUIRE(!cfg->prompt || (cfg->prompt_len >= 1 && !(cfg->lm && cfg->lm_weight != 0.0f) && !cfg->utt_max_steps &&
                               !cfg->utt_min_steps),
              "beam_search: a token prompt excludes the LM scorer and the grouped search");
  SBK_REQUIRE(!cfg->out_probe || (cfg->probe_pos >= 0 && cfg->probe_pos <= pos_off && cfg->probe_token >= 0 &&
                                  cfg->probe_token < W->vocab), "beam_search: probe position / token out of range");
  const bool ctc = cfg->ctc_weight > 0.0f;
  const int topk = cfg->topk > 1 ? cfg->topk : 1;
  SBK_REQUIRE(topk <= cfg->beam, "beam_search: topk %d exceeds the beam %d", topk, cfg->beam);
  SBK_REQUIRE(!ctc || (ctc_w && ctc_b), "beam_search: ctc_weight > 0 needs the ctc_lin weights");
  SBK_REQUIRE(!ctc || (cfg->bos != cfg->eos && cfg->bos != cfg->blank && cfg->eos != cfg->blank),
              "Set blank, eos and bos to different indexes for joint ATT/CTC or CTC decoding");
  SBK_REQUIRE(workspace_bytes >= sbk_beam_search_workspace_bytes(W, cfg, B, T), "beam_search: workspace too small");
  SBK_REQUIRE((reinterpret_cast<uintptr_t>(workspace) & 255) == 0, "beam_search: workspace must be 256-byte aligned");
  hipStream_t st = sbk::as_stream(stream);
  const int beam = cfg->beam, V = W->vocab, n = B * beam, dm = W->d_model;
  const int Lmax = (cfg->max_steps > 0 ? cfg->max_steps : 1) + pos_off;
  if (steps_run) *steps_run = 0;
  if (B == 0) return 0;

  Carver c{static_cast<char*>(workspace), 0, false};
  DecoderBufs d;
  BeamBufs bb;
  carve_decoder(c, d, W, n, B, T, Lmax);
  carve_beam(c, bb, B, beam, T, V, Lmax, ctc, cfg->ctc_window_size);
  const sbk_lm_weights* LM = (cfg->lm && cfg->lm_weight != 0.0f) ? cfg->lm : nullptr;
  LmBufs lb;
  if (LM) {
    SBK_TRY(check_lm(LM));
    SBK_REQUIRE(LM->vocab == V, "beam_search: the LM scores %d tokens, the decoder %d", LM->vocab, V);
    SBK_REQUIRE(cfg->max_steps <= LM->max_len, "beam_search: %d steps exceed the LM positional table", cfg->max_steps);
    SBK_REQUIRE(cfg->lm_temperature > 0.0f, "beam_search: lm_temperature must be positive");
    carve_lm(c, lb, LM, n, Lmax);
  }
  const float* extra = LM ? lb.logits : nullptr;

  const int Vp = ctc_pitch(V);
  SBK_TRY(project_memory(W, d, enc, B, T, st));
  if (ctc) {
    int rc = -1;
    if (cfg->ctc_w3 && sbk::x3_routed(B * T, V, dm))
      rc = sbk::gemm_nt_x3(enc, dm, cfg->ctc_w3, ctc_b, nullptr, 0, bb.ctc_x, Vp, B * T, V, dm, SBK_ACT_NONE, 1.0f, nullptr, 0, st);
    if (rc == -1) rc = sbk::gemm_nt(enc, dm, ctc_w, dm, ctc_b, nullptr, 0, bb.ctc_x, Vp, B * T, V, dm, SBK_ACT_NONE, 1.0f, nullptr, 0, st);
    SBK_TRY(rc);
    SBK_TRY(sbk::log_softmax_rows(bb.ctc_x, bb.ctc_x, B * T, V, 1.0f, 1.0f, st, nullptr, nullptr, Vp));
    SBK_HIP(hipMemsetAsync(bb.phi[1], 0, sbk::ctc_state_floats(B, beam, T) * sizeof(float), st));
    SBK_TRY(sbk::ctc_prepare(bb.ctc_x, bb.ctc_xb, enc_len, bb.phi[0], bb.psi_prev[0], B, T, V, beam, cfg->blank, st, Vp));
  }
  bb.s.pos_off = pos_off;
  SBK_LAUNCH(beam_init_kernel, dim3(sbk::cdiv(n > B ? n : B, 256)), dim3(256), 0, st, bb.s, B, beam, cfg->bos);
  SBK_TRY(sbk::launch_status("beam_init"));
  if (pos_off > 0) {
    SBK_LAUNCH(kv_prompt_init_kernel, dim3(sbk::cdiv(n * pos_off, 256)), dim3(256), 0, st, bb.s, n, Lmax, pos_off);
    for (int p = 0; p < pos_off; ++p) {
      const bool probe = cfg->out_probe && p == cfg->probe_pos;
      SBK_LAUNCH(prompt_col_kernel, dim3(sbk::cdiv(n, 256)), dim3(256), 0, st, cfg->prompt, bb.s.tokens[1], n, beam, pos_off + 1, p);
      SBK_TRY(decoder_step(W, d, bb.s.tokens[1], bb.s.kv_slot[0], enc_len, p, n, B, T, beam, Lmax, probe, st));
      if (probe) {
        SBK_LAUNCH(softmax_prob_kernel, dim3(n), dim3(256), 0, st, (const float*)d.logits, bb.am_max, W->vocab, cfg->probe_token);
        SBK_LAUNCH(probe_pick_kernel, dim3(sbk::cdiv(B, 256)), dim3(256), 0, st, (const float*)bb.am_max, cfg->out_probe, B, beam);
      }
    }
    SBK_LAUNCH(prompt_col_kernel, dim3(sbk::cdiv(n, 256)), dim3(256), 0, st, cfg->prompt, bb.s.tokens[0], n, beam, pos_off + 1, pos_off);
    SBK_TRY(sbk::launch_status("beam_search prompt"));
  }

  const int window = ctc ? cfg->ctc_window_size : 0;
  SBK_REQUIRE(window >= 0 && (window == 0 || (!cfg->utt_max_steps && !cfg->utt_min_steps)),
              "beam_search: ctc_window_size excludes the grouped search");
  if (window > 0) {
    SBK_LAUNCH(win_init_kernel, dim3(sbk::cdiv(Lmax, 256)), dim3(256), 0, st, bb.win, Lmax);
    SBK_TRY(sbk::launch_status("ctc window"));
  }
  const float attn_w = ctc ? 1.0f - cfg->ctc_weight : 1.0f;
  SideStream* side = (ctc && cfg->overlap_ctc && window == 0) ? side_stream() : nullptr;
  const bool psi_aside = side && (cfg->overlap_ctc & 2);
  hipStream_t cst = side ? side->s : st;
  hipStream_t pst = psi_aside ? side->s : st;
  if (ctc && psi_aside) {
    SBK_HIP(hipEventRecord(side->fork, st));
    SBK_HIP(hipStreamWaitEvent(cst, side->fork, 0));
    SBK_TRY(sbk::ctc_psi_step(bb.ctc_x, bb.phi[0], bb.s.tokens[0], enc_len, bb.psi, B, T, V, beam, 0, cfg->blank,
                              cfg->eos, pst, nullptr, 0, Vp));
    SBK_HIP(hipEventRecord(side->join, cst));
  }
  int32_t* step_dev = bb.s.n_full + 2;
  auto issue_step = [&](int step, int cur, bool counter) -> int {
    SBK_TRY(decoder_step(W, d, bb.s.tokens[cur], bb.s.kv_slot[cur], enc_len, pos_off + step, n, B, T, beam, Lmax, true, st));
    if (step == 0 && cfg->out_probe && cfg->probe_pos == pos_off) {
      SBK_LAUNCH(softmax_prob_kernel, dim3(n), dim3(256), 0, st, (const float*)d.logits, bb.am_max, W->vocab, cfg->probe_token);
      SBK_LAUNCH(probe_pick_kernel, dim3(sbk::cdiv(B, 256)), dim3(256), 0, st, (const float*)bb.am_max, cfg->out_probe, B, beam);
    }
    const bool fused = sbk::g_score_fused && beam <= kMaxBeam && V <= 256 * 32 && !(ctc && cfg->ctc_candidates > 0);
    const float ls_temp = cfg->temperature_post ? 1.0f : cfg->temperature;
    const float ls_w = cfg->temperature_post ? attn_w / cfg->temperature : attn_w;
    const float* first_bias = step == 0 ? cfg->first_bias : nullptr;
    if (!fused) {
      SBK_TRY(sbk::log_softmax_rows(d.logits, bb.am, n, V, ls_temp, ls_w, st, cfg->logit_bias, first_bias));
      if (cfg->using_eos_threshold) SBK_TRY(sbk::row_max(bb.am, bb.am_max, n, V, st));
    }
    const int eos_floor = step < cfg->min_steps;
    if (LM) {
      SBK_TRY(lm_step(LM, lb, bb.s.tokens[cur], bb.s.kv_slot[cur], bb.s.seq[cur], Lmax, 1, cfg->bos, step, n, Lmax, st));
      SBK_TRY(sbk::log_softmax_rows(lb.logits, lb.logits, n, V, cfg->lm_temperature, cfg->lm_weight, st));
    }
    const int32_t* win = nullptr;
    if (window > 0) {
      SBK_TRY(sbk::cross_attn_avg_probs(d.q, d.ckv[W->n_layers - 1], enc_len, bb.attn_avg, n, T, dm, W->nhead, beam, st));
      SBK_LAUNCH(attn_peak_kernel, dim3(n), dim3(256), 0, st, (const float*)bb.attn_avg, (const float*)bb.peak_val[cur],
                 (const int32_t*)bb.peak_pos[cur], (const int32_t*)bb.s.parent, bb.peak_val[cur ^ 1], bb.peak_pos[cur ^ 1],
                 bb.win, T, step);
      SBK_TRY(sbk::launch_status("attn_peak"));
      win = bb.win + 2 * step;
    }
    if (ctc) {
      if (side && (psi_aside || step > 0)) SBK_HIP(hipStreamWaitEvent(st, side->join, 0));
      if (!psi_aside)
        SBK_TRY(sbk::ctc_psi_step(bb.ctc_x, bb.phi[cur], bb.s.tokens[cur], enc_len, bb.psi, B, T, V, beam, step,
                                  cfg->blank, cfg->eos, st, win, window, Vp));
      if (fused) {
      } else if (cfg->ctc_candidates > 0) {
        SBK_TRY(sbk::am_only(bb.am, bb.comb, n, V, cfg->eos, eos_floor, cfg->using_eos_threshold, cfg->eos_threshold,
                             cfg->minus_inf, bb.am_max, extra, st, cfg->utt_min_steps, beam, step));
        SBK_TRY(sbk::ctc_partial_combine(bb.comb, bb.topk_val, bb.psi, bb.psi_prev[cur], n, V, cfg->ctc_candidates,
                                         cfg->blank, cfg->eos, cfg->ctc_weight, cfg->minus_inf, st));
      } else {
        SBK_TRY(sbk::ctc_combine(bb.am, bb.am_max, bb.psi, bb.psi_prev[cur], bb.comb, n, V, cfg->blank, cfg->eos,
                                 cfg->ctc_weight, eos_floor, cfg->using_eos_threshold, cfg->eos_threshold,
                                 cfg->minus_inf, extra, st, cfg->utt_min_steps, beam, step));
      }
    } else if (!fused) {
      SBK_TRY(sbk::am_only(bb.am, bb.comb, n, V, cfg->eos, eos_floor, cfg->using_eos_threshold, cfg->eos_threshold,
                           cfg->minus_inf, bb.am_max, extra, st, cfg->utt_min_steps, beam, step));
    }
    const float norm = cfg->length_normalization ? (float)(step + 1) : 0.0f;
    const int32_t* sp = sbk::g_step_ptr;
    const int32_t* umax = cfg->utt_max_steps;
    if (fused) {
      sbk::ProfScope prof("score_topk", 8.0 * n * V, (ctc ? 12.0 : 8.0) * n * V, st);
      ScoreArgs a{d.logits, cfg->logit_bias, first_bias, bb.am, ctc ? bb.psi : nullptr, ctc ? bb.psi_prev[cur] : nullptr,
                  extra, bb.s.seq_scores, bb.topk_val, bb.topk_idx, sp, cfg->utt_min_steps, umax, V, beam, step,
                  cfg->min_steps, eos_floor, cfg->using_eos_threshold, cfg->eos, cfg->blank, 1.0f / ls_temp, ls_w,
                  cfg->ctc_weight, cfg->eos_threshold, cfg->minus_inf, norm};
      if (V <= 256 * 4)
        SBK_LAUNCH(score_topk_row_kernel<4>, dim3(n), dim3(256), 0, st, a);
      else if (V <= 256 * 20)
        SBK_LAUNCH(score_topk_row_kernel<20>, dim3(n), dim3(256), 0, st, a);
      else
        SBK_LAUNCH(score_topk_row_kernel<32>, dim3(n), dim3(256), 0, st, a);
    } else if (beam > kMaxBeam) {
      sbk::ProfScope prof("beam_topk_large", 10.0 * n * V, 20.0 * n * V, st);
      SBK_LAUNCH(beam_topk_large_kernel, dim3(B), dim3(1024), 0, st, (const float*)bb.comb,
                 (const float*)bb.s.seq_scores, bb.s.cand_val, bb.s.cand_idx, V, beam, norm, sp, step, umax);
    } else {
      sbk::ProfScope prof("beam_topk", 2.0 * n * V, 4.0 * n * V, st);
      SBK_LAUNCH(beam_topk_stage1_kernel, dim3(kTopkChunks, B), dim3(256), 0, st, (const float*)bb.comb,
                 (const float*)bb.s.seq_scores, bb.topk_val, bb.topk_idx, V, beam, norm, sp, step, umax);
      SBK_LAUNCH(beam_topk_stage2_kernel, dim3(B), dim3(256), 0, st, (const float*)bb.topk_val,
                 (const int32_t*)bb.topk_idx, bb.s.cand_val, bb.s.cand_idx, beam, sp, step, umax, kTopkChunks);
    }
    SBK_TRY(sbk::launch_status("beam_topk"));
    {
      sbk::ProfScope prof("beam_update", 0.0, 24.0 * n * (step + 1), st);
      if (fused)
        SBK_LAUNCH(beam_merge_update_kernel, dim3(B), dim3(256), 0, st, bb.s, (const float*)bb.topk_val,
                   (const int32_t*)bb.topk_idx, (const float*)bb.am, cur, step, V, beam, Lmax, cfg->eos,
                   cfg->length_normalization, sp, umax, beam);
      else
        SBK_LAUNCH(beam_update_kernel, dim3(B), dim3(256), 0, st, bb.s, (const float*)bb.am, cur, step, V, beam, Lmax,
                   cfg->eos, cfg->length_normalization, sp, umax);
    }
    SBK_TRY(sbk::launch_status("beam_update"));
    if (ctc && (counter || step + 1 < cfg->max_steps)) {
      if (side) {
        SBK_HIP(hipEventRecord(side->fork, st));
        SBK_HIP(hipStreamWaitEvent(cst, side->fork, 0));
      }
      SBK_TRY(sbk::ctc_advance(bb.ctc_x, bb.phi[cur], bb.psi, bb.s.parent, bb.s.tokens[cur ^ 1], bb.s.tokens[cur],
                               bb.phi[cur ^ 1], bb.psi_prev[cur ^ 1], n, T, V, beam, step, cfg->blank, cst, win, window, Vp));
      if (psi_aside)
        SBK_TRY(sbk::ctc_psi_step(bb.ctc_x, bb.phi[cur ^ 1], bb.s.tokens[cur ^ 1], enc_len, bb.psi, B, T, V, beam,
                                  step + 1, cfg->blank, cfg->eos, pst, nullptr, 0, Vp));
      if (side) SBK_HIP(hipEventRecord(side->join, cst));
    }
    if (counter) {
      SBK_LAUNCH(step_inc_kernel, dim3(1), dim3(1), 0, st, step_dev);
      SBK_TRY(sbk::launch_status("step_inc"));
    }
    return 0;
  };
  const bool polling = host_flag && cfg->check_every > 0 && g_poll.begin();
  auto poll_full = [&](int steps_done) -> int {
    if (!(polling && (steps_done % cfg->check_every == 0) && steps_done < cfg->max_steps)) return 0;
    return g_poll.poll(bb.s.n_full, B, st);
  };

  int cur = 0, steps = 0;
  int graph_mode = cfg->graph_mode;
  if (graph_mode && (side || sbk::prof_enabled() || T > 900 || cfg->max_steps < 2 || pos_off > 0 || cfg->first_bias || window > 0)) graph_mode = 0;
  if (graph_mode && sbk::persist_eligible(W, n, B, beam, Lmax)) graph_mode = 0;
  if (graph_mode) {
    struct Scope {
      ~Scope() {
        sbk::g_step_ptr = nullptr;
        if (exec) (void)hipGraphExecDestroy(exec);
        if (graph) (void)hipGraphDestroy(graph);
      }
      hipGraph_t graph = nullptr;
      hipGraphExec_t exec = nullptr;
    } scope;
    SBK_HIP(hipMemsetAsync(step_dev, 0, sizeof(int32_t), st));
    sbk::g_step_ptr = step_dev;
    sbk::g_step_min_steps = cfg->min_steps;
    if (graph_mode == 1) {
      if (hipStreamBeginCapture(st, hipStreamCaptureModeThreadLocal) == hipSuccess) {
        int rc = issue_step(0, 0, true);
        if (!rc) rc = issue_step(0, 1, true);
        const hipError_t e = hipStreamEndCapture(st, &scope.graph);
        if (rc) return rc;
        if (e != hipSuccess || hipGraphInstantiate(&scope.exec, scope.graph, nullptr, nullptr, 0) != hipSuccess) {
          scope.exec = nullptr;
          (void)hipGetLastError();
        }
      } else {
        (void)hipGetLastError();
      }
    }
    const int pairs = cfg->max_steps / 2;
    bool done = false;
    for (int p = 0; p < pairs && !done; ++p) {
      if (scope.exec) {
        SBK_HIP(hipGraphLaunch(scope.exec, st));
      } else {
        SBK_TRY(issue_step(0, 0, true));
        SBK_TRY(issue_step(0, 1, true));
      }
      steps += 2;
      const int r = poll_full(steps);
      if (r < 0) return sbk::fail(1, "beam_search: stop-rule poll failed");
      done = r == 1;
    }
    if (!done && (cfg->max_steps & 1)) {
      SBK_TRY(issue_step(0, 0, true));
      ++steps;
    }
    cur = steps & 1;
  } else {
    for (int step = 0; step < cfg->max_steps; ++step) {
      SBK_TRY(issue_step(step, cur, false));
      cur ^= 1;
      steps = step + 1;
      const int r = poll_full(steps);
      if (r < 0) return sbk::fail(1, "beam_search: stop-rule poll failed");
      if (r == 1) break;
    }
  }
  if (side) SBK_HIP(hipStreamWaitEvent(st, side->join, 0));
  if (steps_run) *steps_run = steps;
  SBK_LAUNCH(beam_finalize_kernel, dim3(B), dim3(256), 0, st, bb.s, cur, steps, beam, Lmax, Lmax - pos_off, topk, out_tokens, out_len,
             out_score, out_logp, cfg->utt_max_steps, out_longest);
  SBK_TRY(sbk::launch_status("beam_finalize"));
  if (out_max_len)
    SBK_HIP(hipMemcpyAsync(out_max_len, bb.s.n_full + 1, sizeof(int32_t), hipMemcpyDeviceToDevice, st));
  return 0;
}

extern "C" size_t sbk_decoder_prefix_workspace_bytes(const sbk_decoder_weights* W, int n, int T, int L) {
  if (!W) return 0;
  Carver c{nullptr, 0, true};
  DecoderBufs d;
  carve_decoder(c, d, W, n, n, T, L);
  c.take<int32_t>((size_t)n * L);
  c.take<int32_t>((size_t)n);
  c.take<int32_t>(64 + 2 * (size_t)n);
  return c.used + 256;
}

__global__ void gather_col_kernel(const int32_t* __restrict__ tokens, int32_t* __restrict__ col, int n, int L, int p) {
  const int i = blockIdx.x * blockDim.x + threadIdx.x;
  if (i < n) col[i] = tokens[(size_t)i * L + p];
}

extern "C" int sbk_decoder_prefix_f32(const sbk_decoder_weights* W, const int32_t* tokens, const float* enc,
                                      const int32_t* enc_len, void* workspace, size_t workspace_bytes, float* pred,
                                      int n, int T, int L, sbk_stream_t stream) {
  SBK_TRY(check_weights(W));
  if (n == 0 || L == 0) return 0;
  SBK_REQUIRE(tokens && enc && enc_len && workspace && pred, "decoder_prefix: null");
  SBK_REQUIRE(L <= W->max_len, "decoder_prefix: prefix longer than the positional table");
  SBK_REQUIRE(workspace_bytes >= sbk_decoder_prefix_workspace_bytes(W, n, T, L), "decoder_prefix: workspace too small");
  hipStream_t st = sbk::as_stream(stream);
  if (n == 0 || L == 0) return 0;
  Carver c{static_cast<char*>(workspace), 0, false};
  DecoderBufs d;
  carve_decoder(c, d, W, n, n, T, L);
  int32_t* kv_slot = c.take<int32_t>((size_t)n * L);
  int32_t* col = c.take<int32_t>((size_t)n);
  int32_t* misc = c.take<int32_t>(64 + 2 * (size_t)n);
  SBK_TRY(project_memory(W, d, enc, n, T, st));
  SBK_LAUNCH(greedy_init_kernel, dim3(sbk::cdiv(n, 256)), dim3(256), 0, st, misc + 64, misc + 64 + n, misc, kv_slot, n, L, 0);
  SBK_TRY(sbk::launch_status("prefix_init"));
  for (int p = 0; p < L; ++p) {
    SBK_LAUNCH(gather_col_kernel, dim3(sbk::cdiv(n, 256)), dim3(256), 0, st, tokens, col, n, L, p);
    SBK_TRY(decoder_step(W, d, col, kv_slot, enc_len, p, n, n, T, 1, L, false, st));
    SBK_LAUNCH(copy_rows_kernel, dim3(n), dim3(256), 0, st, (const float*)d.h, pred + (size_t)p * W->d_model, n,
               W->d_model, (long)L * W->d_model);
    SBK_TRY(sbk::launch_status("prefix_copy"));
  }
  return 0;
}

extern "C" size_t sbk_lm_prefix_workspace_bytes(const sbk_lm_weights* LM, int n, int L) {
  if (!LM) return 0;
  Carver c{nullptr, 0, true};
  LmBufs d;
  carve_lm(c, d, LM, n, L > 0 ? L : 1);
  c.take<int32_t>((size_t)n * (L > 0 ? L : 1));
  c.take<int32_t>((size_t)n);
  c.take<int32_t>(64 + 2 * (size_t)n);
  return c.used + 256;
}

extern "C" int sbk_lm_prefix_f32(const sbk_lm_weights* LM, const int32_t* tokens, void* workspace,
                                 size_t workspace_bytes, float* logits, int n, int L, sbk_stream_t stream) {
  SBK_TRY(check_lm(LM));
  if (n == 0 || L == 0) return 0;
  SBK_REQUIRE(tokens && workspace && logits, "lm_prefix: null");
  SBK_REQUIRE(L <= LM->max_len, "lm_prefix: prefix longer than the positional table");
  SBK_REQUIRE(workspace_bytes >= sbk_lm_prefix_workspace_bytes(LM, n, L), "lm_prefix: workspace too small");
  hipStream_t st = sbk::as_stream(stream);
  if (n == 0 || L == 0) return 0;
  Carver c{static_cast<char*>(workspace), 0, false};
  LmBufs d;
  carve_lm(c, d, LM, n, L);
  int32_t* kv_slot = c.take<int32_t>((size_t)n * L);
  int32_t* col = c.take<int32_t>((size_t)n);
  int32_t* misc = c.take<int32_t>(64 + 2 * (size_t)n);
  SBK_LAUNCH(greedy_init_kernel, dim3(sbk::cdiv(n, 256)), dim3(256), 0, st, misc + 64, misc + 64 + n, misc, kv_slot, n, L, 0);
  SBK_TRY(sbk::launch_status("lm_prefix_init"));
  for (int p = 0; p < L; ++p) {
    SBK_LAUNCH(gather_col_kernel, dim3(sbk::cdiv(n, 256)), dim3(256), 0, st, tokens, col, n, L, p);
    SBK_TRY(lm_step(LM, d, col, kv_slot, tokens, L, 0, 0, p, n, L, st));
    SBK_LAUNCH(copy_rows_kernel, dim3(n), dim3(256), 0, st, (const float*)d.logits, logits + (size_t)p * LM->vocab, n,
               LM->vocab, (long)L * LM->vocab);
    SBK_TRY(sbk::launch_status("lm_prefix_copy"));
  }
  return 0;
}

extern "C" size_t sbk_greedy_search_workspace_bytes(const sbk_decoder_weights* W, int B, int T, int max_steps) {
  if (!W) return 0;
  Carver c{nullptr, 0, true};
  DecoderBufs d;
  const int L = max_steps > 0 ? max_steps : 1;
  carve_decoder(c, d, W, B, B, T, L);
  c.take<int32_t>((size_t)B * L);
  c.take<int32_t>(64 + 2 * (size_t)B);
  return c.used + 256;
}

extern "C" int sbk_greedy_search_f32(const sbk_decoder_weights* W, const float* enc, const int32_t* enc_len,
                                     void* workspace, size_t workspace_bytes, int32_t* out_tokens, float* out_scores,
                                     int32_t* host_flag, int32_t* steps_run, int B, int T, int min_steps, int max_steps,
                                     int bos, int eos, int check_every, sbk_stream_t stream) {
  SBK_TRY(check_weights(W));
  if (B == 0) {
    if (steps_run) *steps_run = 0;
    return 0;
  }
  SBK_REQUIRE(enc && enc_len && workspace && out_tokens && out_scores && W->seq_w && W->seq_b, "greedy_search: null");
  SBK_REQUIRE(max_steps <= W->max_len, "greedy_search: too many steps for the positional table");
  SBK_REQUIRE(workspace_bytes >= sbk_greedy_search_workspace_bytes(W, B, T, max_steps), "greedy: workspace too small");
  hipStream_t st = sbk::as_stream(stream);
  if (steps_run) *steps_run = 0;
  const int L = max_steps > 0 ? max_steps : 1;
  if (B == 0) return 0;
  Carver c{static_cast<char*>(workspace), 0, false};
  DecoderBufs d;
  carve_decoder(c, d, W, B, B, T, L);
  int32_t* kv_slot = c.take<int32_t>((size_t)B * L);
  int32_t* misc = c.take<int32_t>(64 + 2 * (size_t)B);
  int32_t *n_ended = misc, *tok = misc + 64, *ended = misc + 64 + B;
  SBK_TRY(project_memory(W, d, enc, B, T, st));
  SBK_LAUNCH(greedy_init_kernel, dim3(sbk::cdiv(B, 256)), dim3(256), 0, st, tok, ended, n_ended, kv_slot, B, L, bos);
  SBK_TRY(sbk::launch_status("greedy_init"));
  SBK_HIP(hipMemsetAsync(out_tokens, 0, (size_t)B * L * sizeof(int32_t), st));
  SBK_HIP(hipMemsetAsync(out_scores, 0, (size_t)B * L * sizeof(float), st));
  int k = 0;
  const bool polling = host_flag && check_every > 0 && g_poll.begin();
  for (int step = min_steps; step < max_steps; ++step, ++k) {
    SBK_TRY(decoder_step(W, d, tok, kv_slot, enc_len, k, B, B, T, 1, L, true, st));
    SBK_LAUNCH(greedy_pick_kernel, dim3(B), dim3(256), 0, st, (const float*)d.logits, tok, ended, out_tokens,
               out_scores, n_ended, W->vocab, k, L, eos, (const float*)nullptr, (const float*)nullptr);
    SBK_TRY(sbk::launch_status("greedy_pick"));
    if (polling && ((k + 1) % check_every == 0)) {
      const int r = g_poll.poll(n_ended, B, st);
      if (r < 0) return sbk::fail(1, "greedy_search: stop-rule poll failed");
      if (r == 1) {
        ++k;
        break;
      }
    }
  }
  if (steps_run) *steps_run = k;
  return 0;
}

extern "C" size_t sbk_prompted_greedy_search_workspace_bytes(const sbk_decoder_weights* W, int B, int T, int P,
                                                             int max_new) {
  if (!W) return 0;
  Carver c{nullptr, 0, true};
  DecoderBufs d;
  const int L = (P > 0 ? P - 1 : 0) + (max_new > 0 ? max_new : 1);
  carve_decoder(c, d, W, B, B, T, L);
  c.take<int32_t>((size_t)B * L);
  c.take<int32_t>((size_t)B);
  c.take<int32_t>(64 + 2 * (size_t)B);
  return c.used + 256;
}

extern "C" int sbk_prompted_greedy_search_f32(const sbk_decoder_weights* W, const float* enc, const int32_t* enc_len,
                                              const int32_t* prompt, int P, const float* logit_bias,
                                              const float* first_bias, void* workspace, size_t workspace_bytes,
                                              int32_t* out_tokens, float* out_scores, int probe_pos, int probe_token,
                                              float* out_probe, int32_t* host_flag, int32_t* steps_run, int B, int T,
                                              int max_new, int eos, int check_every, sbk_stream_t stream) {
  SBK_TRY(check_weights(W));
  if (steps_run) *steps_run = 0;
  if (B == 0 || max_new <= 0) return 0;
  SBK_REQUIRE(enc && enc_len && prompt && workspace && out_tokens && out_scores && W->seq_w && W->seq_b,
              "prompted_greedy_search: null");
  SBK_REQUIRE(P >= 1, "prompted_greedy_search: the prompt holds at least the first decoder input token");
  const int L = P - 1 + max_new;
  SBK_REQUIRE(L <= W->max_len, "prompted_greedy_search: prompt + new tokens (%d) exceed the positional table (%d)", L,
              W->max_len);
  SBK_REQUIRE(!out_probe || (probe_pos >= 0 && probe_pos < P && probe_token >= 0 && probe_token < W->vocab),
              "prompted_greedy_search: probe position / token out of range");
  SBK_REQUIRE(workspace_bytes >= sbk_prompted_greedy_search_workspace_bytes(W, B, T, P, max_new),
              "prompted_greedy_search: workspace too small");
  hipStream_t st = sbk::as_stream(stream);
  Carver c{static_cast<char*>(workspace), 0, false};
  DecoderBufs d;
  carve_decoder(c, d, W, B, B, T, L);
  int32_t* kv_slot = c.take<int32_t>((size_t)B * L);
  int32_t* col = c.take<int32_t>((size_t)B);
  int32_t* misc = c.take<int32_t>(64 + 2 * (size_t)B);
  int32_t *n_ended = misc, *tok = misc + 64, *ended = misc + 64 + B;
  SBK_TRY(project_memory(W, d, enc, B, T, st));
  SBK_LAUNCH(greedy_init_kernel, dim3(sbk::cdiv(B, 256)), dim3(256), 0, st, tok, ended, n_ended, kv_slot, B, L, 0);
  SBK_TRY(sbk::launch_status("greedy_init"));
  SBK_HIP(hipMemsetAsync(out_tokens, 0, (size_t)B * max_new * sizeof(int32_t), st));
  SBK_HIP(hipMemsetAsync(out_scores, 0, (size_t)B * max_new * sizeof(float), st));
  for (int p = 0; p + 1 < P; ++p) {
    const bool probe = out_probe && p == probe_pos;
    SBK_LAUNCH(gather_col_kernel, dim3(sbk::cdiv(B, 256)), dim3(256), 0, st, prompt, col, B, P, p);
    SBK_TRY(decoder_step(W, d, col, kv_slot, enc_len, p, B, B, T, 1, L, probe, st));
    if (probe) SBK_LAUNCH(softmax_prob_kernel, dim3(B), dim3(256), 0, st, (const float*)d.logits, out_probe, W->vocab, probe_token);
  }
  SBK_LAUNCH(gather_col_kernel, dim3(sbk::cdiv(B, 256)), dim3(256), 0, st, prompt, tok, B, P, P - 1);
  SBK_TRY(sbk::launch_status("prompt"));
  int k = 0;
  const bool polling = host_flag && check_every > 0 && g_poll.begin();
  for (; k < max_new; ++k) {
    SBK_TRY(decoder_step(W, d, tok, kv_slot, enc_len, P - 1 + k, B, B, T, 1, L, true, st));
    if (k == 0 && out_probe && probe_pos == P - 1)
      SBK_LAUNCH(softmax_prob_kernel, dim3(B), dim3(256), 0, st, (const float*)d.logits, out_probe, W->vocab, probe_token);
    SBK_LAUNCH(greedy_pick_kernel, dim3(B), dim3(256), 0, st, (const float*)d.logits, tok, ended, out_tokens, out_scores,
               n_ended, W->vocab, k, max_new, eos, logit_bias, k == 0 ? first_bias : (const float*)nullptr);
    SBK_TRY(sbk::launch_status("greedy_pick"));
    if (polling && ((k + 1) % check_every == 0)) {
      const int r = g_poll.poll(n_ended, B, st);
      if (r < 0) return sbk::fail(1, "greedy_search: stop-rule poll failed");
      if (r == 1) {
        ++k;
        break;
      }
    }
  }
  if (steps_run) *steps_run = k < max_new ? k : max_new;
  return 0;
}
```

Measured before the change: 13070.

## Fuse same-token CTC score into advance and drop full am write in fused scorer

The CTC advance kernel now also builds segment tables in LDS and computes the repeated-token prefix score for the next step, so the separate same-token kernel launch per step is removed and psi_step patches that entry from a small buffer. The fused score/top-k kernel gains a TAIL mode that skips writing the full log-prob row and instead stores only the selected candidates' acoustic scores, which beam update then reads. TAIL is enabled by default by raising g_score_fused to 2. This trades one kernel launch and an n*V store per step for extra LDS work in advance and recomputing log-softmax for the winning candidates.

```diff
diff --git a/speechbrain_amd/csrc/ctc_prefix.hip b/speechbrain_amd/csrc/ctc_prefix.hip
--- a/speechbrain_amd/csrc/ctc_prefix.hip
+++ b/speechbrain_amd/csrc/ctc_prefix.hip
@@ -35,7 +35,8 @@
 
 template <typename Row>
 __device__ __forceinline__ void build_segment_tables(Row row, int T, int lane, float* __restrict__ sg,
-                                                     float* __restrict__ sb, int* __restrict__ se, int bp) {
+                                                     float* __restrict__ sb, int* __restrict__ se, int bp,
+                                                     float* lds_sb = nullptr, int* lds_se = nullptr) {
   const int nseg = nseg_of(T);
   for (int s0 = 0; s0 < nseg; s0 += 2) {
     const int seg = s0 + (lane >> 5);
@@ -47,9 +48,14 @@
     for (int m = 16; m >= 1; m >>= 1) e = max(e, sbk::shfl_xor(e, m));
     if (seg < nseg && t < T) {
       sg[(size_t)t * bp] = sbk::fast_ldexp(v.mg, v.eg - e);
-      sb[t] = sbk::fast_ldexp(v.mb, v.eb - e);
-    }
-    if (seg < nseg && (lane & 31) == 0) se[(size_t)seg * bp] = e;
+      const float vb = sbk::fast_ldexp(v.mb, v.eb - e);
+      sb[t] = vb;
+      if (lds_sb) lds_sb[t] = vb;
+    }
+    if (seg < nseg && (lane & 31) == 0) {
+      se[(size_t)seg * bp] = e;
+      if (lds_se) lds_se[seg] = e;
+    }
   }
 }
 
@@ -127,7 +133,8 @@
 __global__ void __launch_bounds__(256) ctc_score_step_kernel(CtcStepArgs a, const float* __restrict__ P,
                                                              const BF* __restrict__ st, const float* __restrict__ sg,
                                                              const int* __restrict__ se,
-                                                             float* __restrict__ psi_out) {
+                                                             float* __restrict__ psi_out,
+                                                             const float* __restrict__ rep) {
   constexpr int BP = 16;
   constexpr int NV = (NB + 3) / 4;
   SBK_DYN_LDS(float, lds);
@@ -263,6 +270,7 @@
       if (j0 + j < a.beam) {
         const int n = b * a.beam + j0 + j;
         float psi = bf_log(mps[k][j], Eps[k][j]);
+        if (rep && c[k] == a.last_tok[n] && c[k] != a.eos && c[k] != a.blank) psi = rep[n];
         if (c[k] == a.eos) {
           const BF s = st[(size_t)n * T + last_frame];
           psi = bf_log(s.mg, s.eg);
@@ -276,7 +284,8 @@
 
 __global__ void __launch_bounds__(64) ctc_same_token_kernel(CtcStepArgs a, const float* __restrict__ P,
                                                             const BF* __restrict__ st, const float* __restrict__ sb,
-                                                            const int* __restrict__ se, float* __restrict__ psi_out) {
+                                                            const int* __restrict__ se, float* __restrict__ psi_out,
+                                                            float* __restrict__ rep_out) {
   const int n = blockIdx.x, lane = threadIdx.x;
   if (a.step_ptr) a.prefix_len = a.step_ptr[0];
   const int b = n / a.beam, c = a.last_tok[n];
@@ -308,7 +317,12 @@
   for (int k = 32; k >= 1; k >>= 1) Emax = max(Emax, sbk::shfl_xor(Emax, k));
   float v = sbk::fast_ldexp(m, E - Emax);
   v = sbk::wave_sum(v);
-  if (lane == 0) psi_out[(size_t)n * V + c] = bf_log(v, Emax);
+  if (lane == 0) {
+    if (rep_out)
+      rep_out[n] = bf_log(v, Emax);
+    else
+      psi_out[(size_t)n * V + c] = bf_log(v, Emax);
+  }
 }
 
 __global__ void __launch_bounds__(256) ctc_combine_kernel(CtcStepArgs a, const float* __restrict__ am,
@@ -444,8 +458,12 @@
   const int32_t* win;
   int window;
   int ldp;
+  const int32_t* enc_len;
+  float* rep_out;
+  int eos;
 };
 
+template <bool REP>
 __global__ void __launch_bounds__(64) ctc_advance_kernel(CtcAdvArgs a) {
   SBK_DYN_LDS(float, lds);
   if (a.step_ptr) a.prefix_len = a.step_ptr[0];
@@ -518,6 +536,55 @@
     }
   }
   __syncthreads();
+  if constexpr (REP) {
+    auto conv = [&](int t) SBK_INLINE_LAMBDA {
+      BF s;
+      const float g = onb[t] + obl[t];
+      const int kg = sbk::frexp_exp(g), kb = sbk::frexp_exp(obl[t]);
+      s.mg = g > 0.0f ? sbk::fast_ldexp(g, 1 - kg) : 0.0f;
+      s.eg = g > 0.0f ? oe[t] + kg - 1 : kNegE;
+      s.mb = obl[t] > 0.0f ? sbk::fast_ldexp(obl[t], 1 - kb) : 0.0f;
+      s.eb = obl[t] > 0.0f ? oe[t] + kb - 1 : kNegE;
+      return s;
+    };
+    const int nseg = nseg_of(T);
+    const int bp = beam_pitch(a.beam);
+    BF* strow = a.st_new + (size_t)n * T;
+    float* lsb = mph;
+    int* lse = eph;
+    build_segment_tables(
+        [&](int t) SBK_INLINE_LAMBDA {
+          const BF s = conv(t);
+          strow[t] = s;
+          return s;
+        },
+        T, lane, a.sg_new + (size_t)b * T * bp + n % a.beam, a.sb_new + (size_t)n * T,
+        a.se_new + (size_t)b * nseg * bp + n % a.beam, bp, lsb, lse);
+    if (lane == 0) a.psi_prev_new[n] = a.psi[(size_t)p * a.V + c];
+    __syncthreads();
+    if (c == a.eos || c == a.blank || c < 0 || c >= a.V) return;
+    int start, end;
+    ctc_frame_range(a.prefix_len + 1, T, nullptr, 0, &start, &end);
+    end = ctc_clip_to_length(end, a.blank, a.enc_len[b]);
+    float m = 0.0f;
+    int E = kNegE;
+    for (int u = start - 1 + lane; u < end - 1; u += 64) {
+      const float term = lsb[u] * pc[u + 1];
+      const int k = sbk::frexp_exp(term);
+      const int et = term > 0.0f ? lse[u / kSeg] + k : kNegE;
+      const float mt = sbk::fast_ldexp(term, -k);
+      const int E2 = max(E, et);
+      m = sbk::fast_ldexp(m, E - E2) + sbk::fast_ldexp(mt, et - E2);
+      E = E2;
+    }
+    int Emax = E;
+#pragma unroll
+    for (int k = 32; k >= 1; k >>= 1) Emax = max(Emax, sbk::shfl_xor(Emax, k));
+    float v = sbk::fast_ldexp(m, E - Emax);
+    v = sbk::wave_sum(v);
+    if (lane == 0) a.rep_out[n] = bf_log(v, Emax);
+    return;
+  }
   BF* bfrow = reinterpret_cast<BF*>(pc);
   for (int t0 = 0; t0 < T; t0 += 64) {
     const int t = t0 + lane;
@@ -637,7 +704,8 @@
 }
 
 int ctc_psi_step(const float* P, const float* state, const int32_t* last_tok, const int32_t* enc_len, float* psi, int B,
-                 int T, int V, int beam, int prefix_len, int blank, int eos, hipStream_t st, const int32_t* win, int window, int ldp);
+                 int T, int V, int beam, int prefix_len, int blank, int eos, hipStream_t st, const int32_t* win, int window, int ldp,
+                 const float* rep = nullptr);
 
 size_t ctc_state_floats(int B, int beam, int T) {
   const size_t n_bh = (size_t)B * beam, bp = beam_pitch(beam);
@@ -658,7 +726,9 @@
 }
 
 int ctc_psi_step(const float* P, const float* state, const int32_t* last_tok, const int32_t* enc_len, float* psi, int B,
-                 int T, int V, int beam, int prefix_len, int blank, int eos, hipStream_t st, const int32_t* win, int window, int ldp) {
+                 int T, int V, int beam, int prefix_len, int blank, int eos, hipStream_t st, const int32_t* win, int window, int ldp,
+                 const float* rep) {
+  if (rep && win) return fail(SBK_EINVAL, "ctc_psi_step: prepared repeated-token entries exclude the attention window");
   CtcStepArgs a{last_tok, enc_len, B, T, V, beam, prefix_len, blank, eos, 0.0f, 0, 0, 0.0f, 0.0f, g_step_ptr, 0};
   a.win = win;
   a.window = window;
@@ -674,7 +744,7 @@
     if (lds > 64 * 1024 && SBK_ALLOW_DYN_LDS((ctc_score_step_kernel<NB, TP, NT>), lds) != hipSuccess)                    \
       return fail(SBK_EINVAL, "ctc_psi_step: cannot raise the LDS window to %zu B", lds);                               \
     SBK_LAUNCH((ctc_score_step_kernel<NB, TP, NT>), grid, block, lds, st, a, P, (const BF*)v.st, (const float*)v.sg,    \
-               (const int*)v.se, psi);                                                                                  \
+               (const int*)v.se, psi, rep);                                                                             \
   } while (0)
 #define SBK_CTC_LAUNCH_ONE(NB, TP)                                                                                      \
   do {                                                                                                                  \
@@ -697,10 +767,20 @@
 #undef SBK_CTC_LAUNCH_ONE
 #undef SBK_CTC_LAUNCH_NT
   int rc = launch_status("ctc_score_step");
-  if (rc) return rc;
+  if (rc || rep) return rc;
   SBK_LAUNCH(ctc_same_token_kernel, dim3(B * beam), dim3(64), 0, st, a, P, (const BF*)v.st, (const float*)v.sb,
-             (const int*)v.se, psi);
+             (const int*)v.se, psi, (float*)nullptr);
   return launch_status("ctc_same_token");
+}
+
+int ctc_rep_init(const float* P, const float* state, const int32_t* last_tok, const int32_t* enc_len, float* rep, int B, int T,
+                 int V, int beam, int blank, int eos, hipStream_t st, int ldp) {
+  CtcStepArgs a{last_tok, enc_len, B, T, V, beam, 0, blank, eos, 0.0f, 0, 0, 0.0f, 0.0f, nullptr, 0};
+  a.ldp = ldp < V ? V : ldp;
+  const StateView v = view(const_cast<float*>(state), B, beam, T);
+  SBK_LAUNCH(ctc_same_token_kernel, dim3(B * beam), dim3(64), 0, st, a, P, (const BF*)v.st, (const float*)v.sb,
+             (const int*)v.se, (float*)nullptr, rep);
+  return launch_status("ctc_rep_init");
 }
 
 int ctc_combine(const float* am, const float* am_max, const float* psi, const float* psi_prev, float* comb, int n_bh,
@@ -714,15 +794,20 @@
 
 int ctc_advance(const float* P, const float* state_old, const float* psi, const int32_t* parent, const int32_t* token,
                 const int32_t* parent_last_tok, float* state_new, float* psi_prev_new, int n_bh, int T, int V, int beam,
-                int prefix_len, int blank, hipStream_t st, const int32_t* win, int window, int ldp) {
+                int prefix_len, int blank, hipStream_t st, const int32_t* win, int window, int ldp, const int32_t* enc_len,
+                int eos, float* rep_out) {
+  if (rep_out && (win || !enc_len)) return fail(SBK_EINVAL, "ctc_advance: repeated-token entries need enc_len and no attention window");
   const StateView vo = view(const_cast<float*>(state_old), n_bh / beam, beam, T);
   const StateView vn = view(state_new, n_bh / beam, beam, T);
   CtcAdvArgs a{P, vo.st, psi, parent, token, parent_last_tok, vn.st, vn.sg, vn.sb, vn.se, psi_prev_new, n_bh, T, V, beam,
-               prefix_len, blank, g_step_ptr, win, window, ldp < V ? V : ldp};
+               prefix_len, blank, g_step_ptr, win, window, ldp < V ? V : ldp, enc_len, rep_out, eos};
   const size_t lds = (size_t)7 * T * sizeof(float);
   if (lds > 64 * 1024) return fail(SBK_EINVAL, "ctc_advance: T=%d too long for the LDS window", T);
   ProfScope prof("ctc_advance", 14.0 * n_bh * T, 64.0 * n_bh * T, st);
-  SBK_LAUNCH(ctc_advance_kernel, dim3(n_bh), dim3(64), lds, st, a);
+  if (rep_out)
+    SBK_LAUNCH(ctc_advance_kernel<true>, dim3(n_bh), dim3(64), lds, st, a);
+  else
+    SBK_LAUNCH(ctc_advance_kernel<false>, dim3(n_bh), dim3(64), lds, st, a);
   return launch_status("ctc_advance");
 }
 
@@ -829,7 +914,8 @@
   const ScorerWs w = carve_scorer(ws, B, T, V, beam);
   const int cur = step & 1;
   return sbk::ctc_advance(x, w.phi[cur], w.psi, parent, token, parent_last_tok, w.phi[cur ^ 1], w.psi_prev[cur ^ 1], B * beam, T, V,
-                          beam, step, blank, sbk::as_stream(stream), ctc_window_size > 0 ? attn_window : nullptr, ctc_window_size, V);
+                          beam, step, blank, sbk::as_stream(stream), ctc_window_size > 0 ? attn_window : nullptr, ctc_window_size, V,
+                          nullptr, -1, nullptr);
 }
 
 extern "C" int sbk_prof_ctc_psi_repeat_f32(float* P_logsoftmax, const int32_t* enc_len, const int32_t* last_tok,
diff --git a/speechbrain_amd/csrc/search.hip b/speechbrain_amd/csrc/search.hip
--- a/speechbrain_amd/csrc/search.hip
+++ b/speechbrain_amd/csrc/search.hip
@@ -56,7 +56,9 @@
 size_t ctc_state_floats(int B, int beam, int T);
 int ctc_psi_step(const float* P, const float* state, const int32_t* last_tok, const int32_t* enc_len, float* psi, int B,
                  int T, int V, int beam, int prefix_len, int blank, int eos, hipStream_t st, const int32_t* win = nullptr,
-                 int window = 0, int ldp = 0);
+                 int window = 0, int ldp = 0, const float* rep = nullptr);
+int ctc_rep_init(const float* P, const float* state, const int32_t* last_tok, const int32_t* enc_len, float* rep, int B, int T,
+                 int V, int beam, int blank, int eos, hipStream_t st, int ldp);
 int cross_attn_avg_probs(const float* q, const float* kv, const int32_t* enc_len, float* out, int n, int T, int d, int H,
                          int beam, hipStream_t st);
 int ctc_combine(const float* am, const float* am_max, const float* psi, const float* psi_prev, float* comb, int n_bh,
@@ -64,14 +66,15 @@
                 const float* extra, hipStream_t st, const int32_t* utt_min = nullptr, int beam = 1, int step = 0);
 int ctc_advance(const float* x, const float* phi_old, const float* psi, const int32_t* parent, const int32_t* token,
                 const int32_t* parent_last_tok, float* phi_new, float* psi_prev_new, int n_bh, int T, int V, int beam,
-                int prefix_len, int blank, hipStream_t st, const int32_t* win = nullptr, int window = 0, int ldp = 0);
+                int prefix_len, int blank, hipStream_t st, const int32_t* win = nullptr, int window = 0, int ldp = 0,
+                const int32_t* enc_len = nullptr, int eos = -1, float* rep_out = nullptr);
 int am_only(const float* am, float* comb, int n_bh, int V, int eos, int eos_floor, int use_thr, float thr,
             float minus_inf, const float* am_max, const float* extra, hipStream_t st, const int32_t* utt_min = nullptr,
             int beam = 1, int step = 0);
 int row_max(const float* x, float* out, int rows, int V, hipStream_t st);
 int ctc_partial_combine(float* comb, float* thr, const float* psi, const float* psi_prev, int n_bh, int V, int k, int blank,
                         int eos, float weight, float minus_inf, hipStream_t st);
-int g_score_fused = 1;
+int g_score_fused = 2;
 }
 
 namespace {
@@ -230,6 +233,7 @@
   const float* seq;
   float* pval;
   int32_t* pidx;
+  float* pam;
   const int32_t* step_ptr;
   const int32_t* utt_min;
   const int32_t* utt_max;
@@ -237,9 +241,10 @@
   float inv_temp, w, ctc_weight, thr, minus_inf, norm;
 };
 
-template <int NPT>
+template <int NPT, bool TAIL>
 __global__ void __launch_bounds__(256) score_topk_row_kernel(ScoreArgs a) {
-  __shared__ float red[4];
+  __shared__ float red_s[TAIL ? 3 : 1][4];
+  float* red = red_s[0];
   __shared__ float wv[4][kMaxBeam];
   __shared__ int wi[4][kMaxBeam];
   const int n = blockIdx.x, tid = threadIdx.x, lane = tid & 63, wave = tid >> 6;
@@ -272,7 +277,7 @@
   if (lane == 0) red[wave] = m;
   __syncthreads();
   m = fmaxf(fmaxf(red[0], red[1]), fmaxf(red[2], red[3]));
-  __syncthreads();
+  if constexpr (TAIL) red = red_s[1]; else __syncthreads();
   float s = 0.0f;
 #pragma unroll
   for (int i = 0; i < NPT; ++i)
@@ -281,16 +286,19 @@
   if (lane == 0) red[wave] = s;
   __syncthreads();
   const float lse = sbk::add_rn(m, logf((red[0] + red[1]) + (red[2] + red[3])));
-  __syncthreads();
+  if constexpr (TAIL) red = red_s[2]; else __syncthreads();
   float am_max = -INFINITY;
 #pragma unroll
   for (int i = 0; i < NPT; ++i) {
     const int c = tid + 256 * i;
     if (c < V) {
       x[i] = sbk::ls_out(x[i], lse, a.w);
-      a.am[ro + c] = x[i];
+      if constexpr (!TAIL) a.am[ro + c] = x[i];
       am_max = fmaxf(am_max, x[i]);
     }
+  }
+  if constexpr (TAIL) {
+    if (j == 0 && tid == 0) a.pam[(size_t)b * kTopkChunks * (kMaxBeam + 1) + kMaxBeam] = x[0];
   }
   if (a.use_thr) {
     am_max = sbk::wave_max(am_max);
@@ -366,6 +374,7 @@
     }
     float* ov_ = a.pval + ((size_t)b * kTopkChunks + j) * kMaxBeam;
     int32_t* oi_ = a.pidx + ((size_t)b * kTopkChunks + j) * kMaxBeam;
+    int won = INT_MAX;
     for (int r = 0; r < k; ++r) {
       float wbv = v;
       int wbi = i2;
@@ -374,9 +383,17 @@
         ov_[r] = wbv;
         oi_[r] = wbi;
       }
+      if (lane == r) won = wbi;
       if (i2 == wbi && wbi != INT_MAX) {
         v = -INFINITY;
         i2 = INT_MAX;
+      }
+    }
+    if constexpr (TAIL) {
+      if (won != INT_MAX) {
+        const int c = won - j * V;
+        const float xl = sbk::ls_logit(a.logits[ro + c], a.bias ? a.bias[c] : 0.0f, a.bias2 ? a.bias2[c] : 0.0f, a.inv_temp);
+        a.pam[((size_t)b * kTopkChunks + j) * (kMaxBeam + 1) + lane] = sbk::ls_out(xl, lse, a.w);
       }
     }
   }
@@ -584,7 +601,16 @@
 
 __device__ __forceinline__ void beam_update_body(const BeamState& s, const float* __restrict__ am, int cur, int step, int V,
                                                  int beam, int Lmax, int eos, int length_norm,
-                                                 const int32_t* __restrict__ utt_max) {
+                                                 const int32_t* __restrict__ utt_max,
+                                                 const int32_t* __restrict__ pidx = nullptr,
+                                                 const float* __restrict__ pam = nullptr) {
+  auto am_of = [&](int pred, int tok, int cand) SBK_INLINE_LAMBDA -> float {
+    if (!pam) return am[(size_t)pred * V + tok];
+    const size_t row = (size_t)blockIdx.x * kTopkChunks + cand / V;
+    for (int r = 0; r < beam; ++r)
+      if (pidx[row * kMaxBeam + r] == cand) return pam[row * (kMaxBeam + 1) + r];
+    return pam[(size_t)blockIdx.x * kTopkChunks * (kMaxBeam + 1) + kMaxBeam];
+  };
   __shared__ int h_src[kMaxBeamLarge];
   __shared__ int h_dst[kMaxBeamLarge];
   __shared__ int h_n;
@@ -616,7 +642,7 @@
       s.kv_slot[nxt][o + s.pos_off] = s.kv_slot[cur][po + s.pos_off];
     } else {
       s.seq[nxt][o] = tok;
-      s.lp[nxt][o] = am[(size_t)pred * V + tok];
+      s.lp[nxt][o] = am_of(pred, tok, cand);
       s.kv_slot[nxt][o + s.pos_off] = pred;
       s.tokens[nxt][n] = tok;
       s.parent[n] = pred;
@@ -651,7 +677,7 @@
     const size_t fo = ((size_t)b * beam + h_dst[k]) * Lmax;
     for (int p = tid; p <= step; p += 256) {
       s.fin_seq[fo + p] = p < step ? s.seq[cur][(size_t)pred * Lmax + p] : tok;
-      s.fin_lp[fo + p] = p < step ? s.lp[cur][(size_t)pred * Lmax + p] : am[(size_t)pred * V + tok];
+      s.fin_lp[fo + p] = p < step ? s.lp[cur][(size_t)pred * Lmax + p] : am_of(pred, tok, cand);
     }
   }
 }
@@ -669,7 +695,8 @@
                                                                 const float* __restrict__ am, int cur, int step, int V,
                                                                 int beam, int Lmax, int eos, int length_norm,
                                                                 const int32_t* __restrict__ step_ptr,
-                                                                const int32_t* __restrict__ utt_max, int nchunks) {
+                                                                const int32_t* __restrict__ utt_max, int nchunks,
+                                                                const float* __restrict__ pam) {
   const int b = blockIdx.x;
   if (step_ptr) step = step_ptr[0];
   if (!(utt_max && step >= utt_max[b])) {
@@ -684,7 +711,7 @@
     if (threadIdx.x < beam && s.cand_idx[b * beam + threadIdx.x] == INT_MAX) s.cand_idx[b * beam + threadIdx.x] = 0;
     __syncthreads();
   }
-  beam_update_body(s, am, cur, step, V, beam, Lmax, eos, length_norm, utt_max);
+  beam_update_body(s, am, cur, step, V, beam, Lmax, eos, length_norm, utt_max, pam ? pidx : nullptr, pam);
 }
 
 __global__ void __launch_bounds__(256) beam_finalize_kernel(BeamState s, int cur, int steps_done, int beam, int Lmax,
@@ -1122,7 +1149,9 @@
 struct BeamBufs {
   BeamState s;
   float *am, *comb, *psi, *am_max, *ctc_x, *ctc_xb, *phi[2], *psi_prev[2];
+  float* psi_rep[2];
   float* topk_val;
+  float* topk_am;
   int32_t* topk_idx;
   float* attn_avg;
   float* peak_val[2];
@@ -1197,6 +1226,7 @@
   b.am_max = c.take<float>(n);
   b.topk_val = c.take<float>((size_t)B * kTopkChunks * kMaxBeam);
   b.topk_idx = c.take<int32_t>((size_t)B * kTopkChunks * kMaxBeam);
+  b.topk_am = c.take<float>((size_t)B * kTopkChunks * (kMaxBeam + 1));
   if (ctc) {
     b.psi = c.take<float>(n * V);
     b.ctc_x = c.take<float>((size_t)B * T * ctc_pitch(V));
@@ -1204,6 +1234,7 @@
     for (int k = 0; k < 2; ++k) {
       b.phi[k] = c.take<float>(sbk::ctc_state_floats(B, beam, T));
       b.psi_prev[k] = c.take<float>(n);
+      b.psi_rep[k] = c.take<float>(n);
     }
     if (window > 0) {
       b.attn_avg = c.take<float>(n * T);
@@ -1323,6 +1354,12 @@
     SBK_LAUNCH(win_init_kernel, dim3(sbk::cdiv(Lmax, 256)), dim3(256), 0, st, bb.win, Lmax);
     SBK_TRY(sbk::launch_status("ctc window"));
   }
+  const bool fused = sbk::g_score_fused && beam <= kMaxBeam && V <= 256 * 32 && !(ctc && cfg->ctc_candidates > 0);
+  const bool tail = fused && sbk::g_score_fused >= 2;
+  const bool rep = tail && ctc && window == 0;
+  if (rep)
+    SBK_TRY(sbk::ctc_rep_init(bb.ctc_x, bb.phi[0], bb.s.tokens[0], enc_len, bb.psi_rep[0], B, T, V, beam, cfg->blank, cfg->eos,
+                              st, Vp));
   const float attn_w = ctc ? 1.0f - cfg->ctc_weight : 1.0f;
   SideStream* side = (ctc && cfg->overlap_ctc && window == 0) ? side_stream() : nullptr;
   const bool psi_aside = side && (cfg->overlap_ctc & 2);
@@ -1332,7 +1369,7 @@
     SBK_HIP(hipEventRecord(side->fork, st));
     SBK_HIP(hipStreamWaitEvent(cst, side->fork, 0));
     SBK_TRY(sbk::ctc_psi_step(bb.ctc_x, bb.phi[0], bb.s.tokens[0], enc_len, bb.psi, B, T, V, beam, 0, cfg->blank,
-                              cfg->eos, pst, nullptr, 0, Vp));
+                              cfg->eos, pst, nullptr, 0, Vp, rep ? bb.psi_rep[0] : nullptr));
     SBK_HIP(hipEventRecord(side->join, cst));
   }
   int32_t* step_dev = bb.s.n_full + 2;
@@ -1342,7 +1379,6 @@
       SBK_LAUNCH(softmax_prob_kernel, dim3(n), dim3(256), 0, st, (const float*)d.logits, bb.am_max, W->vocab, cfg->probe_token);
       SBK_LAUNCH(probe_pick_kernel, dim3(sbk::cdiv(B, 256)), dim3(256), 0, st, (const float*)bb.am_max, cfg->out_probe, B, beam);
     }
-    const bool fused = sbk::g_score_fused && beam <= kMaxBeam && V <= 256 * 32 && !(ctc && cfg->ctc_candidates > 0);
     const float ls_temp = cfg->temperature_post ? 1.0f : cfg->temperature;
     const float ls_w = cfg->temperature_post ? attn_w / cfg->temperature : attn_w;
     const float* first_bias = step == 0 ? cfg->first_bias : nullptr;
@@ -1368,7 +1404,7 @@
       if (side && (psi_aside || step > 0)) SBK_HIP(hipStreamWaitEvent(st, side->join, 0));
       if (!psi_aside)
         SBK_TRY(sbk::ctc_psi_step(bb.ctc_x, bb.phi[cur], bb.s.tokens[cur], enc_len, bb.psi, B, T, V, beam, step,
-                                  cfg->blank, cfg->eos, st, win, window, Vp));
+                                  cfg->blank, cfg->eos, st, win, window, Vp, rep ? bb.psi_rep[cur] : nullptr));
       if (fused) {
       } else if (cfg->ctc_candidates > 0) {
         SBK_TRY(sbk::am_only(bb.am, bb.comb, n, V, cfg->eos, eos_floor, cfg->using_eos_threshold, cfg->eos_threshold,
@@ -1388,17 +1424,25 @@
     const int32_t* sp = sbk::g_step_ptr;
     const int32_t* umax = cfg->utt_max_steps;
     if (fused) {
-      sbk::ProfScope prof("score_topk", 8.0 * n * V, (ctc ? 12.0 : 8.0) * n * V, st);
+      sbk::ProfScope prof("score_topk", 8.0 * n * V, ((ctc ? 12.0 : 8.0) - (tail ? 4.0 : 0.0)) * n * V, st);
       ScoreArgs a{d.logits, cfg->logit_bias, first_bias, bb.am, ctc ? bb.psi : nullptr, ctc ? bb.psi_prev[cur] : nullptr,
-                  extra, bb.s.seq_scores, bb.topk_val, bb.topk_idx, sp, cfg->utt_min_steps, umax, V, beam, step,
+                  extra, bb.s.seq_scores, bb.topk_val, bb.topk_idx, bb.topk_am, sp, cfg->utt_min_steps, umax, V, beam, step,
                   cfg->min_steps, eos_floor, cfg->using_eos_threshold, cfg->eos, cfg->blank, 1.0f / ls_temp, ls_w,
                   cfg->ctc_weight, cfg->eos_threshold, cfg->minus_inf, norm};
+#define SBK_SCORE_LAUNCH(NPT)                                                      \
+  do {                                                                             \
+    if (tail)                                                                      \
+      SBK_LAUNCH((score_topk_row_kernel<NPT, true>), dim3(n), dim3(256), 0, st, a);  \
+    else                                                                           \
+      SBK_LAUNCH((score_topk_row_kernel<NPT, false>), dim3(n), dim3(256), 0, st, a); \
+  } while (0)
       if (V <= 256 * 4)
-        SBK_LAUNCH(score_topk_row_kernel<4>, dim3(n), dim3(256), 0, st, a);
+        SBK_SCORE_LAUNCH(4);
       else if (V <= 256 * 20)
-        SBK_LAUNCH(score_topk_row_kernel<20>, dim3(n), dim3(256), 0, st, a);
+        SBK_SCORE_LAUNCH(20);
       else
-        SBK_LAUNCH(score_topk_row_kernel<32>, dim3(n), dim3(256), 0, st, a);
+        SBK_SCORE_LAUNCH(32);
+#undef SBK_SCORE_LAUNCH
     } else if (beam > kMaxBeam) {
       sbk::ProfScope prof("beam_topk_large", 10.0 * n * V, 20.0 * n * V, st);
       SBK_LAUNCH(beam_topk_large_kernel, dim3(B), dim3(1024), 0, st, (const float*)bb.comb,
@@ -1416,7 +1460,7 @@
       if (fused)
         SBK_LAUNCH(beam_merge_update_kernel, dim3(B), dim3(256), 0, st, bb.s, (const float*)bb.topk_val,
                    (const int32_t*)bb.topk_idx, (const float*)bb.am, cur, step, V, beam, Lmax, cfg->eos,
-                   cfg->length_normalization, sp, umax, beam);
+                   cfg->length_normalization, sp, umax, beam, tail ? (const float*)bb.topk_am : (const float*)nullptr);
       else
         SBK_LAUNCH(beam_update_kernel, dim3(B), dim3(256), 0, st, bb.s, (const float*)bb.am, cur, step, V, beam, Lmax,
                    cfg->eos, cfg->length_normalization, sp, umax);
@@ -1428,10 +1472,11 @@
         SBK_HIP(hipStreamWaitEvent(cst, side->fork, 0));
       }
       SBK_TRY(sbk::ctc_advance(bb.ctc_x, bb.phi[cur], bb.psi, bb.s.parent, bb.s.tokens[cur ^ 1], bb.s.tokens[cur],
-                               bb.phi[cur ^ 1], bb.psi_prev[cur ^ 1], n, T, V, beam, step, cfg->blank, cst, win, window, Vp));
+                               bb.phi[cur ^ 1], bb.psi_prev[cur ^ 1], n, T, V, beam, step, cfg->blank, cst, win, window, Vp,
+                               enc_len, cfg->eos, rep ? bb.psi_rep[cur ^ 1] : nullptr));
       if (psi_aside)
         SBK_TRY(sbk::ctc_psi_step(bb.ctc_x, bb.phi[cur ^ 1], bb.s.tokens[cur ^ 1], enc_len, bb.psi, B, T, V, beam,
-                                  step + 1, cfg->blank, cfg->eos, pst, nullptr, 0, Vp));
+                                  step + 1, cfg->blank, cfg->eos, pst, nullptr, 0, Vp, rep ? bb.psi_rep[cur ^ 1] : nullptr));
       if (side) SBK_HIP(hipEventRecord(side->join, cst));
     }
     if (counter) {
```

New measurement: 13020 (median of 3 runs). Within noise of the previous version (-0.4%).
